# yangdongchao/RSTnet

Measured on NVIDIA H100. Metric: codec_frames_per_s, higher is better.
Workload: dtype f32

## Files before the change

### include/rstnet_b200.h

```cpp
#ifndef RSTNET_B200_H
#define RSTNET_B200_H

#include <stdint.h>

#ifdef __cplusplus
extern "C" {
#endif

typedef void* rstnet_stream_t;

enum { RSTNET_ACT_NONE = 0, RSTNET_ACT_ELU = 1, RSTNET_ACT_GELU = 2 };

int rstnet_version(void);
const char* rstnet_last_error(void);
int64_t rstnet_launch_count(void);
uint32_t rstnet_device_error_flags(int clear);

typedef struct {
  const float* A;
  int64_t a_batch_stride, a_row_stride;
  const float* Wt;
  const float* bias;
  const float* scale;
  const float* R;
  int64_t r_batch_stride, r_row_stride;
  float* C;
  int64_t c_batch_stride, c_row_stride;
  int32_t batch, rows, N, K;
  int32_t pre_act, post_act;
  int32_t taps;
  int64_t tap_stride;
} rstnet_gemm_rows_args;
int rstnet_gemm_rows_f32(const rstnet_gemm_rows_args* args, rstnet_stream_t stream);

typedef struct rstnet_tc_plan rstnet_tc_plan;
typedef struct {
  const float* A;
  int64_t a_i_stride, a_o_stride;
  int32_t a_c_extent, a_i_extent, a_o_extent;
  int32_t taps, tap_di, tap_do, o_mul;
  const float* W;
  const float* W_lo;
  int32_t N, Kc;
  int32_t I_out, O_out;
  float* C;
  int64_t c_i_stride, c_o_stride, c_split_stride;
  const float* R;
  int64_t r_i_stride, r_o_stride, r_split_stride;
  const float* bias;
  const float* scale;
  int32_t n_split;
  int32_t pre_act, post_act, precision;
  float* C2;
  int32_t act2;
} rstnet_tc_gemm_desc;
int rstnet_tc_gemm_create(const rstnet_tc_gemm_desc* desc, rstnet_tc_plan** out);
int rstnet_tc_gemm_run(const rstnet_tc_plan* plan, rstnet_stream_t stream);
void rstnet_tc_gemm_destroy(rstnet_tc_plan* plan);
int rstnet_tc_gemm_grid(const rstnet_tc_plan* plan, int32_t* grid_x, int32_t* grid_y, int32_t* tile_n);
int rstnet_tc_gemm_create_ex(const rstnet_tc_gemm_desc* desc, int32_t kpair, rstnet_tc_plan** out);
int rstnet_tc_gemm_kpair(const rstnet_tc_plan* plan, int32_t* on);
typedef struct rstnet_tc_resblock_plan rstnet_tc_resblock_plan;
typedef struct {
  const float* Y;
  int64_t y_i_stride, y_o_stride;
  int32_t channels;
  int32_t I_out, O_out, y_rows;
  const float* W1;
  const float* W1_lo;
  const float* b1;
  const float* W2;
  const float* W2_lo;
  const float* b2;
  float* out;
  int64_t out_i_stride, out_o_stride;
} rstnet_tc_resblock_desc;
int rstnet_tc_resblock_create(const rstnet_tc_resblock_desc* desc, rstnet_tc_resblock_plan** out);
int rstnet_tc_resblock_run(const rstnet_tc_resblock_plan* plan, rstnet_stream_t stream);
void rstnet_tc_resblock_destroy(rstnet_tc_resblock_plan* plan);

int rstnet_tf32_split_f32(const float* x, float* hi, float* lo, int64_t n, rstnet_stream_t stream);

int rstnet_conv1d_cin1_f32(const float* x, int64_t x_batch_stride, int64_t x_time_stride, const float* w, const float* bias,
                           float* out, float* out2 , int64_t out_batch_stride,
                           int64_t out_time_stride, int32_t batch, int32_t T, int32_t Cout, int32_t k,
                           int32_t post_act, int32_t act2, rstnet_stream_t stream);

int rstnet_conv1d_cout1_f32(const float* x, int64_t x_batch_stride, int64_t x_time_stride, const float* w,
                            const float* bias, float* out, int64_t out_batch_stride, int32_t batch,
                            int32_t T, int32_t Cin, int32_t k, rstnet_stream_t stream);

int rstnet_convtr1d_depthwise_f32(const float* x, int64_t x_batch_stride, int64_t x_time_stride,
                                  const float* w, float* out, int64_t out_batch_stride,
                                  int64_t out_time_stride, int32_t batch, int32_t T, int32_t C,
                                  int32_t stride, rstnet_stream_t stream);

int rstnet_rows_fill_f32(float* buf, int64_t batch_stride, int32_t batch, int32_t C, int32_t row0,
                         int32_t nrows, int32_t mode, int32_t src_row, const int64_t* only_if_zero,
                         int32_t only_if_zero_stride ,
                         int32_t channels_per_stream, rstnet_stream_t stream);
int rstnet_rows_fill_tail_f32(float* buf, int64_t batch_stride, int32_t batch, int32_t C, int32_t row0, int32_t nrows,
                              int32_t mode, const int64_t* valid, int64_t valid_div, int32_t channels_per_stream,
                              rstnet_stream_t stream);
typedef struct {
  float* buf;
  int64_t batch_stride;
  int32_t C, src_row, dst_row, nrows;
  int32_t cps;
  int32_t reserved;
} rstnet_row_copy;
int rstnet_rows_copy_table_f32(const rstnet_row_copy* table_dev, int32_t n_entries, int32_t batch,
                               const int64_t* active, rstnet_stream_t stream);
int rstnet_counter_add(int64_t* counter, int64_t delta, int32_t n, const int64_t* active ,
                       rstnet_stream_t stream);
int rstnet_counter_add_rows(int64_t* counter, const int64_t* delta, int32_t n, rstnet_stream_t stream);

int rstnet_layer_norm_f32(const float* x, int64_t x_batch_stride, const float* weight, const float* bias,
                          float* y, int32_t batch, int32_t rows_per_batch, int32_t dim, float eps,
                          rstnet_stream_t stream);

int rstnet_rope_kv_append_f32(float* qkv, int64_t q_batch_stride, int64_t q_time_stride, float* kv,
                              const int64_t* offset, int32_t offset_stride, const float* freqs, int32_t batch,
                              int32_t T, int32_t H, int32_t D, int32_t cap, rstnet_stream_t stream);
int rstnet_ring_attention_f32(const float* qkv, int64_t q_batch_stride, int64_t q_time_stride,
                              const float* kv, const int64_t* offset, int32_t offset_stride, float* out,
                              int64_t o_batch_stride, int64_t o_time_stride, int32_t batch, int32_t T,
                              int32_t H, int32_t D, int32_t cap, int32_t context, int32_t linear,
                              rstnet_stream_t stream);
int rstnet_rope_ring_attention_f32(const float* qkv, int64_t q_batch_stride, int64_t q_time_stride, float* kv,
                                   const int64_t* offset, int32_t offset_stride, const float* freqs, float* out,
                                   int64_t o_batch_stride, int64_t o_time_stride, int32_t batch, int32_t T, int32_t H,
                                   int32_t D, int32_t cap, int32_t context, rstnet_stream_t stream);

int64_t rstnet_rvq_encode_workspace(int64_t N, int32_t n_q, int32_t dim, int32_t bins);
int rstnet_rvq_encode_f32(const float* x, int64_t ldx, const float* E, const float* Et,
                          const float* enorm, int64_t* codes, void* work, int64_t N, int32_t T,
                          int32_t n_q, int32_t n_q_semantic, int32_t dim, int32_t bins,
                          int32_t time_major, rstnet_stream_t stream);
int rstnet_rvq_decode_gather_f32(const int64_t* codes, const float* E, float* q, int64_t N, int32_t T,
                                 int32_t n_q, int32_t n_q_semantic, int32_t dim, int32_t bins,
                                 int32_t time_major, rstnet_stream_t stream);

#define RSTNET_RESAMPLE_MAX_TABLE_BYTES (48 * 1024)
int rstnet_resample_f32(const float* x, int64_t x_row_stride, int64_t x_len, int64_t x_shift, const float* taps,
                        const int32_t* start, int32_t n, int32_t o, int32_t S, int32_t start_max, float* out,
                        int64_t out_row_stride, int64_t out_len, int32_t rows, rstnet_stream_t stream);

#define RSTNET_STFT_FRAMES_PER_BLOCK 16
int64_t rstnet_stft_loss_workspace(int32_t clips, int64_t max_len, int32_t hop);
int rstnet_stft_loss_sums_f32(const float* ref, const float* deg, const int64_t* offsets, const int64_t* lengths,
                              int32_t clips, int64_t min_len, int64_t max_len, int32_t n_fft, int32_t hop, int32_t win,
                              const float* twiddle, const float* window, double* sums, int32_t n_res, int32_t res,
                              void* ws, int64_t ws_bytes, rstnet_stream_t stream);

#define RSTNET_SISNR_SAMPLES_PER_BLOCK 8192
int64_t rstnet_sisnr_moments_workspace(int32_t clips, int64_t max_len);
int rstnet_sisnr_moments_f32(const float* ref, const float* deg, const int64_t* offsets, const int64_t* lengths,
                             int32_t clips, int64_t max_len, double* moments, void* ws, int64_t ws_bytes,
                             rstnet_stream_t stream);


typedef struct rstnet_skinny_plan rstnet_skinny_plan;
int64_t rstnet_skinny_gemm_workspace(int32_t M, int32_t N, int32_t max_splits);
int rstnet_skinny_gemm_create(const void* X, const void* W, const void* R, void* out, float* partial_ws,
                              int32_t M, int32_t N, int32_t K, int32_t max_splits, rstnet_skinny_plan** plan);
int rstnet_skinny_gemm_create_fused(const void* X, const void* W, const void* R, void* out, float* partial_ws,
                                    int32_t M, int32_t N, int32_t K, int32_t max_splits, int32_t fin_mode,
                                    const void* norm_w, void* aux_out, float eps, int32_t kyutai,
                                    rstnet_skinny_plan** plan);
int rstnet_skinny_gemm_run(const rstnet_skinny_plan* plan, rstnet_stream_t stream);
void rstnet_skinny_gemm_destroy(rstnet_skinny_plan* plan);

int rstnet_lm_embed_sum_bf16(const int64_t* seq, int32_t seq_stride, const void* wte, int64_t wte_rows,
                             const void* const* tables_dev, int64_t table_rows, int32_t n_q, int32_t E, void* x, int32_t rows,
                             rstnet_stream_t stream);
int rstnet_lm_embed_rows_bf16(const int64_t* ids, int32_t id_stride, const void* table, int64_t table_rows, int32_t D,
                              void* out, int32_t rows, rstnet_stream_t stream);
int rstnet_lm_rms_norm_bf16(const void* x, const void* w, void* y, int32_t rows, int32_t dim, float eps, int32_t kyutai,
                            rstnet_stream_t stream);
int rstnet_lm_rope_kv_append_bf16(const void* qkv, const void* cos_tab, const void* sin_tab, int64_t rope_rows, int32_t rope_n,
                                  const int64_t* offset, int32_t offset_stride ,
                                  const int32_t* row_stream, const int32_t* row_tl, void* q_out, void* kv, int32_t rows,
                                  int32_t B, int32_t n_head, int32_t n_kv, int32_t hs, int32_t cap, rstnet_stream_t stream);
#define RSTNET_KV_LOG2_PAGE_MIN 4
#define RSTNET_KV_LOG2_PAGE_MAX 12
int rstnet_lm_rope_kv_append_paged_bf16(const void* qkv, const void* cos_tab, const void* sin_tab, int64_t rope_rows,
                                        int32_t rope_n, const int64_t* offset, int32_t offset_stride, const int32_t* row_stream,
                                        const int32_t* row_tl, void* q_out, void* kv, int32_t rows, int32_t B, int32_t n_head,
                                        int32_t n_kv, int32_t hs, int32_t cap, const int32_t* page_table, int32_t pages_stride,
                                        int32_t log2_page, rstnet_stream_t stream);
int rstnet_lm_rope_pair_kv_append_bf16(const void* qkv, const int64_t* offset, int32_t offset_stride, void* q_out, void* kv,
                                       int32_t rows, int32_t B, int32_t H, int32_t hd, int32_t cap, const float* freqs,
                                       rstnet_stream_t stream);
int rstnet_lm_ring_decode_attention_bf16(const void* q, const void* kv, const int64_t* offset, int32_t offset_stride,
                                         const int32_t* row_stream, const int32_t* row_tl, void* out, int32_t rows, int32_t B,
                                         int32_t n_head, int32_t n_kv, int32_t hs, int32_t cap, int32_t context,
                                         rstnet_stream_t stream);
int rstnet_lm_paged_decode_attention_bf16(const void* q, const void* kv, const int64_t* offset, int32_t offset_stride,
                                          const int32_t* row_stream, const int32_t* row_tl, void* out, int32_t rows, int32_t B,
                                          int32_t n_head, int32_t n_kv, int32_t hs, int32_t cap, int32_t context,
                                          const int32_t* page_table, int32_t pages_stride, int32_t log2_page,
                                          rstnet_stream_t stream);
int rstnet_lm_silu_mul_bf16(const void* ab, void* out, int32_t M, int32_t I, rstnet_stream_t stream);
int rstnet_lm_depth_attention_bf16(const void* qkv, void* kvd, void* out, int32_t B, int32_t H, int32_t hd, int32_t cap,
                                   int32_t step, int32_t ring_quirk, rstnet_stream_t stream);
int rstnet_lm_sample_params_bf16(const void* logits, int32_t rows, int32_t V, int32_t n_valid, const int32_t* n_valid_rows,
                                 int32_t n_valid_stride, int32_t top_k, float temp, float top_p, const int32_t* top_k_rows,
                                 const float* temp_rows, const float* top_p_rows, int32_t param_stride, uint32_t seed,
                                 const int64_t* step_counter, const int64_t* step_rows, const uint32_t* key_rows,
                                 int64_t* tokens, int32_t tok_stride, rstnet_stream_t stream);

int rstnet_lm_cross_entropy_bf16(const void* logits, int64_t row_stride, int32_t rows, int32_t V, int32_t groups,
                                 const int64_t* labels, const int64_t* ignore_ids, const float* weights,
                                 const int32_t* row_slot, int32_t n_slots, float* nll, int32_t* pred, double* acc,
                                 rstnet_stream_t stream);

int rstnet_lm_delay_cache_in(int64_t* cache, const int64_t* off, const int64_t* active, const int64_t* delays,
                             const int64_t* user, int32_t user_stride, int64_t* seq, int32_t seq_stride, int32_t B, int32_t K,
                             int32_t dep_q, int32_t CT, int64_t text_init, int64_t audio_init, rstnet_stream_t stream);
int rstnet_lm_delay_cache_out(int64_t* cache, int64_t* off, const int64_t* active, const int64_t* delays,
                              const int64_t* tokens, int32_t tok_stride, int64_t* out, int32_t out_stride, int64_t* valid,
                              int32_t B, int32_t K, int32_t dep_q, int32_t CT, int32_t max_delay, rstnet_stream_t stream);

#ifdef __cplusplus
}
#endif
#endif
```

### rstnet_b200/_lib.py

```python
from __future__ import annotations

import ctypes as C
import os

_HERE = os.path.dirname(os.path.abspath(__file__))
LIB_PATH = os.path.join(_HERE, "lib", "librstnet_b200.so")

ACT_NONE, ACT_ELU, ACT_GELU = 0, 1, 2

SYMBOLS = [
    "rstnet_version", "rstnet_last_error", "rstnet_launch_count", "rstnet_device_error_flags",
    "rstnet_gemm_rows_f32", "rstnet_tc_gemm_create", "rstnet_tc_gemm_run", "rstnet_tc_gemm_destroy", "rstnet_tc_gemm_grid",
    "rstnet_tc_gemm_create_ex", "rstnet_tc_gemm_kpair",
    "rstnet_tc_resblock_create", "rstnet_tc_resblock_run", "rstnet_tc_resblock_destroy", "rstnet_tf32_split_f32", "rstnet_conv1d_cin1_f32", "rstnet_conv1d_cout1_f32",
    "rstnet_convtr1d_depthwise_f32", "rstnet_rows_fill_f32", "rstnet_rows_copy_table_f32",
    "rstnet_counter_add", "rstnet_layer_norm_f32", "rstnet_rope_kv_append_f32",
    "rstnet_ring_attention_f32", "rstnet_rope_ring_attention_f32", "rstnet_rvq_encode_workspace", "rstnet_rvq_encode_f32",
    "rstnet_rvq_decode_gather_f32",
    "rstnet_skinny_gemm_workspace", "rstnet_skinny_gemm_create", "rstnet_skinny_gemm_create_fused", "rstnet_skinny_gemm_run", "rstnet_skinny_gemm_destroy",
    "rstnet_lm_embed_sum_bf16", "rstnet_lm_embed_rows_bf16", "rstnet_lm_rms_norm_bf16", "rstnet_lm_rope_kv_append_bf16",
    "rstnet_lm_rope_pair_kv_append_bf16",
    "rstnet_lm_ring_decode_attention_bf16", "rstnet_lm_silu_mul_bf16", "rstnet_lm_depth_attention_bf16",
    "rstnet_resample_f32", "rstnet_lm_delay_cache_in", "rstnet_lm_delay_cache_out", "rstnet_counter_add_rows",
    "rstnet_lm_cross_entropy_bf16", "rstnet_rows_fill_tail_f32", "rstnet_lm_sample_params_bf16",
    "rstnet_lm_rope_kv_append_paged_bf16", "rstnet_lm_paged_decode_attention_bf16",
    "rstnet_stft_loss_workspace", "rstnet_stft_loss_sums_f32", "rstnet_sisnr_moments_workspace", "rstnet_sisnr_moments_f32",
]

KV_LOG2_PAGE_MIN, KV_LOG2_PAGE_MAX = 4, 12

RESAMPLE_MAX_TABLE_BYTES = 48 * 1024

STFT_FRAMES_PER_BLOCK = 16
SISNR_SAMPLES_PER_BLOCK = 8192


class GemmRowsArgs(C.Structure):
    _fields_ = [
        ("A", C.c_void_p), ("a_batch_stride", C.c_int64), ("a_row_stride", C.c_int64),
        ("Wt", C.c_void_p), ("bias", C.c_void_p), ("scale", C.c_void_p),
        ("R", C.c_void_p), ("r_batch_stride", C.c_int64), ("r_row_stride", C.c_int64),
        ("C", C.c_void_p), ("c_batch_stride", C.c_int64), ("c_row_stride", C.c_int64),
        ("batch", C.c_int32), ("rows", C.c_int32), ("N", C.c_int32), ("K", C.c_int32),
        ("pre_act", C.c_int32), ("post_act", C.c_int32), ("taps", C.c_int32), ("tap_stride", C.c_int64),
    ]


class TcGemmDesc(C.Structure):
    _fields_ = [
        ("A", C.c_void_p), ("a_i_stride", C.c_int64), ("a_o_stride", C.c_int64),
        ("a_c_extent", C.c_int32), ("a_i_extent", C.c_int32), ("a_o_extent", C.c_int32),
        ("taps", C.c_int32), ("tap_di", C.c_int32), ("tap_do", C.c_int32), ("o_mul", C.c_int32),
        ("W", C.c_void_p), ("W_lo", C.c_void_p), ("N", C.c_int32), ("Kc", C.c_int32), ("I_out", C.c_int32), ("O_out", C.c_int32),
        ("C", C.c_void_p), ("c_i_stride", C.c_int64), ("c_o_stride", C.c_int64), ("c_split_stride", C.c_int64),
        ("R", C.c_void_p), ("r_i_stride", C.c_int64), ("r_o_stride", C.c_int64), ("r_split_stride", C.c_int64),
        ("bias", C.c_void_p), ("scale", C.c_void_p),
        ("n_split", C.c_int32), ("pre_act", C.c_int32), ("post_act", C.c_int32), ("precision", C.c_int32),
        ("C2", C.c_void_p), ("act2", C.c_int32),
    ]


class TcResblockDesc(C.Structure):
    _fields_ = [
        ("Y", C.c_void_p), ("y_i_stride", C.c_int64), ("y_o_stride", C.c_int64),
        ("channels", C.c_int32), ("I_out", C.c_int32), ("O_out", C.c_int32), ("y_rows", C.c_int32),
        ("W1", C.c_void_p), ("W1_lo", C.c_void_p), ("b1", C.c_void_p),
        ("W2", C.c_void_p), ("W2_lo", C.c_void_p), ("b2", C.c_void_p),
        ("out", C.c_void_p), ("out_i_stride", C.c_int64), ("out_o_stride", C.c_int64),
    ]


class RowCopy(C.Structure):
    _fields_ = [("buf", C.c_void_p), ("batch_stride", C.c_int64), ("C", C.c_int32), ("src_row", C.c_int32),
                ("dst_row", C.c_int32), ("nrows", C.c_int32), ("cps", C.c_int32), ("reserved", C.c_int32)]


class RstnetError(RuntimeError):
    pass


_lib = None


def lib() -> C.CDLL:
    global _lib
    if _lib is not None:
        return _lib
    if not os.path.exists(LIB_PATH):
        raise RstnetError(
            f"{LIB_PATH} not found: the CUDA extension is not built. Run `python -m rstnet_b200.build` "
            "(there is no CPU fallback).")
    from . import build as _build
    stamp = os.path.join(os.path.dirname(LIB_PATH), "build.sha256")
    if os.path.isdir(_build.CSRC) and (not os.path.exists(stamp) or open(stamp).read().strip() != _build._digest()):
        raise RstnetError(
            f"{LIB_PATH} is stale (built from different sources than rstnet_b200/csrc + include/). "
            "Run `python -m rstnet_b200.build`.")
    L = C.CDLL(LIB_PATH)
    vp, i32, i64, f32 = C.c_void_p, C.c_int32, C.c_int64, C.c_float
    L.rstnet_version.restype = C.c_int
    L.rstnet_last_error.restype = C.c_char_p
    L.rstnet_launch_count.restype = i64
    L.rstnet_gemm_rows_f32.argtypes = [C.POINTER(GemmRowsArgs), vp]
    L.rstnet_tc_gemm_create.argtypes = [C.POINTER(TcGemmDesc), C.POINTER(C.c_void_p)]
    L.rstnet_tc_gemm_run.argtypes = [vp, vp]
    L.rstnet_tc_gemm_destroy.argtypes = [vp]
    L.rstnet_tc_gemm_destroy.restype = None
    L.rstnet_tc_gemm_grid.argtypes = [vp, C.POINTER(i32), C.POINTER(i32), C.POINTER(i32)]
    L.rstnet_tc_gemm_create_ex.argtypes = [C.POINTER(TcGemmDesc), i32, C.POINTER(C.c_void_p)]
    L.rstnet_tc_gemm_kpair.argtypes = [vp, C.POINTER(i32)]
    L.rstnet_tc_resblock_create.argtypes = [C.POINTER(TcResblockDesc), C.POINTER(C.c_void_p)]
    L.rstnet_tc_resblock_run.argtypes = [vp, vp]
    L.rstnet_tc_resblock_destroy.argtypes = [vp]
    L.rstnet_tc_resblock_destroy.restype = None
    L.rstnet_tf32_split_f32.argtypes = [vp, vp, vp, i64, vp]
    L.rstnet_conv1d_cin1_f32.argtypes = [vp, i64, i64, vp, vp, vp, vp, i64, i64, i32, i32, i32, i32, i32, i32, vp]
    L.rstnet_conv1d_cout1_f32.argtypes = [vp, i64, i64, vp, vp, vp, i64, i32, i32, i32, i32, vp]
    L.rstnet_convtr1d_depthwise_f32.argtypes = [vp, i64, i64, vp, vp, i64, i64, i32, i32, i32, i32, vp]
    L.rstnet_rows_fill_f32.argtypes = [vp, i64, i32, i32, i32, i32, i32, i32, vp, i32, i32, vp]
    L.rstnet_rows_fill_tail_f32.argtypes = [vp, i64, i32, i32, i32, i32, i32, vp, i64, i32, vp]
    L.rstnet_rows_copy_table_f32.argtypes = [vp, i32, i32, vp, vp]
    L.rstnet_counter_add.argtypes = [vp, i64, i32, vp, vp]
    L.rstnet_layer_norm_f32.argtypes = [vp, i64, vp, vp, vp, i32, i32, i32, f32, vp]
    L.rstnet_rope_kv_append_f32.argtypes = [vp, i64, i64, vp, vp, i32, vp, i32, i32, i32, i32, i32, vp]
    L.rstnet_ring_attention_f32.argtypes = [vp, i64, i64, vp, vp, i32, vp, i64, i64, i32, i32, i32, i32, i32, i32, i32, vp]
    L.rstnet_rope_ring_attention_f32.argtypes = [vp, i64, i64, vp, vp, i32, vp, vp, i64, i64, i32, i32, i32, i32, i32, i32, vp]
    L.rstnet_rvq_encode_workspace.argtypes = [i64, i32, i32, i32]
    L.rstnet_rvq_encode_workspace.restype = i64
    L.rstnet_rvq_encode_f32.argtypes = [vp, i64, vp, vp, vp, vp, vp, i64, i32, i32, i32, i32, i32, i32, vp]
    L.rstnet_rvq_decode_gather_f32.argtypes = [vp, vp, vp, i64, i32, i32, i32, i32, i32, i32, vp]
    L.rstnet_skinny_gemm_workspace.argtypes = [i32, i32, i32]
    L.rstnet_skinny_gemm_workspace.restype = i64
    L.rstnet_skinny_gemm_create.argtypes = [vp, vp, vp, vp, vp, i32, i32, i32, i32, C.POINTER(C.c_void_p)]
    L.rstnet_skinny_gemm_create_fused.argtypes = [vp, vp, vp, vp, vp, i32, i32, i32, i32, i32, vp, vp, f32, i32, C.POINTER(C.c_void_p)]
    L.rstnet_skinny_gemm_run.argtypes = [vp, vp]
    L.rstnet_skinny_gemm_destroy.argtypes = [vp]
    L.rstnet_skinny_gemm_destroy.restype = None
    L.rstnet_lm_embed_sum_bf16.argtypes = [vp, i32, vp, i64, vp, i64, i32, i32, vp, i32, vp]
    L.rstnet_lm_embed_rows_bf16.argtypes = [vp, i32, vp, i64, i32, vp, i32, vp]
    L.rstnet_device_error_flags.argtypes = [i32]
    L.rstnet_device_error_flags.restype = C.c_uint32
    L.rstnet_lm_rms_norm_bf16.argtypes = [vp, vp, vp, i32, i32, f32, i32, vp]
    L.rstnet_lm_rope_kv_append_bf16.argtypes = [vp, vp, vp, i64, i32, vp, i32, vp, vp, vp, vp, i32, i32, i32, i32, i32, i32, vp]
    L.rstnet_lm_rope_pair_kv_append_bf16.argtypes = [vp, vp, i32, vp, vp, i32, i32, i32, i32, i32, vp, vp]
    L.rstnet_lm_ring_decode_attention_bf16.argtypes = [vp, vp, vp, i32, vp, vp, vp, i32, i32, i32, i32, i32, i32, i32, vp]
    L.rstnet_lm_rope_kv_append_paged_bf16.argtypes = [vp, vp, vp, i64, i32, vp, i32, vp, vp, vp, vp, i32, i32, i32, i32, i32, i32,
                                                      vp, i32, i32, vp]
    L.rstnet_lm_paged_decode_attention_bf16.argtypes = [vp, vp, vp, i32, vp, vp, vp, i32, i32, i32, i32, i32, i32, i32, vp, i32, i32,
                                                        vp]
    L.rstnet_lm_silu_mul_bf16.argtypes = [vp, vp, i32, i32, vp]
    L.rstnet_lm_depth_attention_bf16.argtypes = [vp, vp, vp, i32, i32, i32, i32, i32, i32, vp]
    L.rstnet_resample_f32.argtypes = [vp, i64, i64, i64, vp, vp, i32, i32, i32, i32, vp, i64, i64, i32, vp]
    L.rstnet_lm_delay_cache_in.argtypes = [vp, vp, vp, vp, vp, i32, vp, i32, i32, i32, i32, i32, i64, i64, vp]
    L.rstnet_lm_delay_cache_out.argtypes = [vp, vp, vp, vp, vp, i32, vp, i32, vp, i32, i32, i32, i32, i32, vp]
    L.rstnet_counter_add_rows.argtypes = [vp, vp, i32, vp]
    L.rstnet_lm_cross_entropy_bf16.argtypes = [vp, i64, i32, i32, i32, vp, vp, vp, vp, i32, vp, vp, vp, vp]
    L.rstnet_lm_sample_params_bf16.argtypes = [vp, i32, i32, i32, vp, i32, i32, f32, f32, vp, vp, vp, i32, C.c_uint32, vp, vp, vp,
                                               vp, i32, vp]
    L.rstnet_stft_loss_workspace.argtypes = [i32, i64, i32]
    L.rstnet_stft_loss_workspace.restype = i64
    L.rstnet_stft_loss_sums_f32.argtypes = [vp, vp, vp, vp, i32, i64, i64, i32, i32, i32, vp, vp, vp, i32, i32, vp, i64, vp]
    L.rstnet_sisnr_moments_workspace.argtypes = [i32, i64]
    L.rstnet_sisnr_moments_workspace.restype = i64
    L.rstnet_sisnr_moments_f32.argtypes = [vp, vp, vp, vp, i32, i64, vp, vp, i64, vp]
    for name in SYMBOLS:
        fn = getattr(L, name)
        if fn.restype is C.c_int and name not in ("rstnet_version",):
            pass
    _lib = L
    return L


def check(rc: int, what: str = "") -> None:
    if rc != 0:
        msg = lib().rstnet_last_error()
        raise RstnetError(f"{what or 'rstnet call'} failed (rc={rc}): {msg.decode() if msg else '?'}")


def launch_count() -> int:
    return int(lib().rstnet_launch_count())
```

### rstnet_b200/csrc/gemm_tc.cu

```cuda
#include <cstdlib>

#include "common.cuh"
#include "tc_common.cuh"
#include "../../include/rstnet_b200.h"

namespace rstnet {
extern void count_launch();
using namespace tc;

constexpr int TC_BM = 128;
constexpr int TC_BKE = 32;
constexpr int TC_A_BYTES = TC_BM * 128;
constexpr int TC_CONSUMER_WARPS = 8;
constexpr int TC_THREADS = 32 * TC_CONSUMER_WARPS + 32;
constexpr int TC_CHUNK_STAGES = 4;

struct TcParams {
  float* C;
  float* C2;
  int act2;
  long long c_i_stride, c_o_stride, c_split_stride;
  const float* R;
  long long r_i_stride, r_o_stride, r_split_stride;
  const float* bias;
  const float* scale;
  int n_split;
  int I_out, O_out, N, Kc;
  int taps, tap_di, tap_do, o_mul, kchunks;
  int pre_act, post_act, i_tiles;
  int m_tiles, n_tiles;
  int kpair;
};

template <int BN, int PREC>
struct TcCfg {
  static constexpr bool SPLIT = PREC == 0;
  static constexpr int B_BYTES = BN * 128;
  static constexpr int STAGE_BYTES = TC_A_BYTES + B_BYTES * (SPLIT ? 2 : 1);
  static constexpr int STAGES = (200 * 1024 / STAGE_BYTES) > 8 ? 8 : (200 * 1024 / STAGE_BYTES);
  static constexpr int SMEM_BYTES = STAGES * STAGE_BYTES + 1024  + 256 ;
  static constexpr int Q_PIECES = BN / 32;
  static_assert(STAGES % 2 == 0 && 2 * Q_PIECES <= STAGES, "K-pair rings and queue");
};

__device__ __forceinline__ float tf32_rna(float x) {
  const uint32_t u = __float_as_uint(x);
  return __uint_as_float((x != x ? u | 0x00400000u : u + 0x1000u) & 0xFFFFE000u);
}
__device__ __forceinline__ float tf32_rna_lo(float x, float hi) {
  const float d = x - hi;
  return d != d ? 0.f : __uint_as_float((__float_as_uint(d) + 0x1000u) & 0xFFFFE000u);
}

__device__ __forceinline__ float act_tc(float x, int act) {
  if (act == ACT_ELU) return elu_fast(x);
  if (act == ACT_GELU) return gelu_f(x);
  return x;
}

template <bool SPLIT, bool PRE_ELU>
__device__ __forceinline__ void tc_build_a(uint32_t st, uint32_t a_row, uint32_t a_sw, uint32_t (&ah)[4][4], uint32_t (&al)[4][4]) {
#pragma unroll
  for (int k = 0; k < 4; ++k) {
#pragma unroll
    for (int e = 0; e < 4; ++e) {
      const uint32_t chunk = (uint32_t)(2 * k + (e >> 1));
      float v;
      asm volatile("ld.shared.f32 %0, [%1];" : "=f"(v) : "r"(st + a_row + (e & 1) * 1024u + ((chunk ^ a_sw) << 4)));
      if (PRE_ELU) {
        const float e = __expf(v) - 1.f;
        v = v > 0.f ? v : e;
      }
      if (SPLIT) {
        const bool nonfinite = !(fabsf(v) < INFINITY);
        const float h = nonfinite ? 0.f : __uint_as_float((__float_as_uint(v) + 0x1000u) & 0xFFFFE000u);
        const float d = v - h;
        ah[k][e] = __float_as_uint(h);
        al[k][e] = (__float_as_uint(d) + (nonfinite ? 0u : 0x1000u)) & 0xFFFFE000u;
      } else {
        ah[k][e] = __float_as_uint(tf32_rna(v));
      }
    }
  }
}

template <int BN, bool SPLIT>
__device__ __forceinline__ void tc_mma_stage(float (&d0)[BN / 2], float (&d1)[BN / 2], const uint32_t (&ah)[4][4],
                                             const uint32_t (&al)[4][4], uint64_t db, uint64_t dbl, bool first) {
#pragma unroll
  for (int k = 0; k < 4; ++k) {
    const uint32_t acc_in = (first && k == 0) ? 0u : 1u;
    wgmma_tf32_rs<BN>(d0, ah[k], db + (uint64_t)(2 * k), acc_in);
    if (SPLIT) {
      wgmma_tf32_rs<BN>(d1, al[k], db + (uint64_t)(2 * k), acc_in);
      wgmma_tf32_rs<BN>(d1, ah[k], dbl + (uint64_t)(2 * k), 1u);
    }
  }
}

template <int BN, int PREC, bool PRE_ELU, bool KP>
__global__ void __launch_bounds__(TC_THREADS, 1)
gemm_tc_kernel(const __grid_constant__ CUtensorMap tmA, const __grid_constant__ CUtensorMap tmW,
               const __grid_constant__ CUtensorMap tmWlo, const TcParams p) {
  using Cfg = TcCfg<BN, PREC>;
  constexpr int S = Cfg::STAGES;
  constexpr int CH = TC_CHUNK_STAGES;
  constexpr int NR = BN / 2;
  extern __shared__ uint8_t smem_raw[];
  uint8_t* smem = smem_raw + ((1024u - (smem_u32(smem_raw) & 1023u)) & 1023u);
  uint64_t* full = reinterpret_cast<uint64_t*>(smem + S * Cfg::STAGE_BYTES);
  uint64_t* empty = full + S;
  uint64_t* qfull = empty + S;
  uint64_t* qempty = qfull + 2;
  const int warp = threadIdx.x / 32, lane = threadIdx.x % 32;
  const int total_k = p.taps * p.kchunks;
  const int total_tiles = p.m_tiles * p.n_tiles;
  const int bm = KP ? TC_BM / 2 : TC_BM;
  const int R = KP ? S / 2 : S;

  if (threadIdx.x == 0) {
    for (int s = 0; s < S; ++s) {
      mbar_init(&full[s], 1);
      mbar_init(&empty[s], KP ? TC_CONSUMER_WARPS / 2 : TC_CONSUMER_WARPS);
    }
    for (int q = 0; q < 2; ++q) {
      mbar_init(&qfull[q], 128);
      mbar_init(&qempty[q], 128);
    }
    fence_barrier_init();
  }
  __syncthreads();

  if (warp == TC_CONSUMER_WARPS) {
    if (elect_one()) {
      tma_prefetch_desc(&tmA);
      tma_prefetch_desc(&tmW);
      if (Cfg::SPLIT) tma_prefetch_desc(&tmWlo);
      int pos0 = 0, ph0 = 0, pos1 = 0, ph1 = 0;
      for (int t = blockIdx.x; t < total_tiles; t += gridDim.x) {
        const int nt = t % p.n_tiles, mt = t / p.n_tiles;
        const int i0 = (mt % p.i_tiles) * bm, ot = mt / p.i_tiles, n0 = nt * BN;
        for (int kit = 0; kit < total_k; ++kit) {
          const int w = KP ? (kit / TC_CHUNK_STAGES) & 1 : 0;
          const int pos = w ? pos1 : pos0, ph = w ? ph1 : ph0;
          const int s = w * R + pos;
          const int npos = pos + 1 == R ? 0 : pos + 1, nph = ph ^ (npos == 0);
          if (w) { pos1 = npos; ph1 = nph; } else { pos0 = npos; ph0 = nph; }
          mbar_wait(&empty[s], ph ^ 1);
          const int tap = kit / p.kchunks, kc = kit % p.kchunks;
          uint8_t* st = smem + s * Cfg::STAGE_BYTES;
          mbar_arrive_expect_tx(&full[s], Cfg::STAGE_BYTES - (TC_BM - bm) * 128);
          tma_load_3d(st, &tmA, &full[s], kc * TC_BKE, i0 + tap * p.tap_di, ot * p.o_mul + tap * p.tap_do);
          tma_load_2d(st + TC_A_BYTES, &tmW, &full[s], kit * TC_BKE, n0);
          if (Cfg::SPLIT) tma_load_2d(st + TC_A_BYTES + Cfg::B_BYTES, &tmWlo, &full[s], kit * TC_BKE, n0);
        }
      }
    }
    return;
  }

  const int wg = warp / 4, wq = warp % 4, gq = lane / 4, tq = lane % 4;
  const int r0 = (KP ? 0 : wg * 64) + wq * 16 + gq;
  const uint32_t a_row = (uint32_t)r0 * 128u + (uint32_t)tq * 4u, a_sw = (uint32_t)(r0 & 7);
  const uint32_t smem0 = smem_u32(smem);
  float acc[NR], d0[NR], d1[NR];
#pragma unroll
  for (int j = 0; j < NR; ++j) d0[j] = d1[j] = 0.f;
  const int nch = (total_k + CH - 1) / CH;
  const bool sender = KP && wg == 1;
  auto qel = [&](int q, int j) {
    return reinterpret_cast<float*>(smem + (q * Cfg::Q_PIECES + j / 16) * Cfg::STAGE_BYTES + TC_A_BYTES / 2) +
           (j % 16) * 128 + (threadIdx.x & 127);
  };
  int qn = 0;
  auto take_queued = [&]() {
    mbar_wait(&qfull[qn & 1], (qn >> 1) & 1);
#pragma unroll
    for (int j = 0; j < NR; ++j) acc[j] += *qel(qn & 1, j);
    mbar_arrive(&qempty[qn & 1]);
    ++qn;
  };
  const int base = KP ? wg * R : 0;
  int pos = 0, ph = 0;
  for (int t = blockIdx.x; t < total_tiles; t += gridDim.x) {
    const int nt = t % p.n_tiles, mt = t / p.n_tiles;
    const int i0 = (mt % p.i_tiles) * bm, ot = mt / p.i_tiles, n0 = nt * BN;
#pragma unroll
    for (int j = 0; j < NR; ++j) acc[j] = 0.f;
    for (int c = KP ? wg : 0; c < nch; c += KP ? 2 : 1) {
      const int k0 = c * CH;
      const int nst = total_k - k0 < CH ? total_k - k0 : CH;
      for (int u = 0; u < nst; ++u) {
        const int s = base + pos;
        mbar_wait(&full[s], ph);
        const uint32_t st = smem0 + (uint32_t)(s * Cfg::STAGE_BYTES);
        uint32_t ah[4][4], al[4][4];
        tc_build_a<Cfg::SPLIT, PRE_ELU>(st, a_row, a_sw, ah, al);
        const uint64_t db = gmma_desc_sw128(st + TC_A_BYTES);
        const uint64_t dbl = gmma_desc_sw128(st + TC_A_BYTES + Cfg::B_BYTES);
        wgmma_fence();
        tc_mma_stage<BN, Cfg::SPLIT>(d0, d1, ah, al, db, dbl, u == 0);
        wgmma_commit();
        wgmma_wait<0>();
        __syncwarp();
        if (lane == 0) mbar_arrive(&empty[s]);
        pos = pos + 1 == R ? 0 : pos + 1;
        ph ^= pos == 0;
      }
      fence_acc(d0);
      if (Cfg::SPLIT) fence_acc(d1);
      if (sender) {
        mbar_wait(&qempty[qn & 1], ((qn >> 1) & 1) ^ 1);
#pragma unroll
        for (int j = 0; j < NR; ++j) *qel(qn & 1, j) = Cfg::SPLIT ? d0[j] + d1[j] : d0[j];
        mbar_arrive(&qfull[qn & 1]);
        ++qn;
      } else {
        if (KP && c > 0) take_queued();
#pragma unroll
        for (int j = 0; j < NR; ++j) acc[j] += Cfg::SPLIT ? d0[j] + d1[j] : d0[j];
      }
    }
    if (KP && !sender && nch % 2 == 0) take_queued();
    if (sender) continue;
#pragma unroll
    for (int h = 0; h < 2; ++h) {
      const int i = i0 + r0 + 8 * h;
      if (i >= p.I_out) continue;
      float* crow = p.C + (long long)ot * p.c_o_stride + (long long)i * p.c_i_stride;
      float* crow2 = p.C2 ? p.C2 + (long long)ot * p.c_o_stride + (long long)i * p.c_i_stride : nullptr;
      const float* rrow = p.R ? p.R + (long long)ot * p.r_o_stride + (long long)i * p.r_i_stride : nullptr;
#pragma unroll
      for (int b = 0; b < BN / 8; ++b) {
        const int n = n0 + 8 * b + 2 * tq;
        if (n < p.N) {
          float2 v = make_float2(acc[4 * b + 2 * h], acc[4 * b + 2 * h + 1]);
          if (p.bias) {
            const float2 bb = *reinterpret_cast<const float2*>(p.bias + n);
            v.x += bb.x; v.y += bb.y;
          }
          if (p.scale) {
            const float2 ss = *reinterpret_cast<const float2*>(p.scale + n);
            v.x *= ss.x; v.y *= ss.y;
          }
          long long coff = n, roff = n;
          if (p.n_split > 0) {
            const int j = n / p.n_split, co = n % p.n_split;
            coff = (long long)j * p.c_split_stride + co;
            roff = (long long)j * p.r_split_stride + co;
          }
          if (rrow) {
            const float2 rr = *reinterpret_cast<const float2*>(rrow + roff);
            v.x += rr.x; v.y += rr.y;
          }
          if (crow2)
            *reinterpret_cast<float2*>(crow2 + coff) = make_float2(act_tc(v.x, p.act2), act_tc(v.y, p.act2));
          *reinterpret_cast<float2*>(crow + coff) = make_float2(act_tc(v.x, p.post_act), act_tc(v.y, p.post_act));
        }
      }
    }
  }
}

constexpr int RB_B_BYTES = 64 * 128;
constexpr int RB_STAGE_BYTES = TC_A_BYTES + 2 * RB_B_BYTES;
constexpr int RB_STAGES = 6;

struct RbParams {
  float* out;
  long long o_i_stride, o_o_stride;
  const float* b1;
  const float* b2;
  int I_out, i_tiles, m_tiles;
};

template <int C>
struct RbCfg {
  static constexpr int N1 = C / 2;
  static constexpr int KCH = C / 32;
  static constexpr int P1 = 3 * KCH;
  static constexpr int NS = C / 64;
  static constexpr int K2 = N1 / 32;
  static constexpr int H_BYTES = K2 * TC_A_BYTES;
  static constexpr int SMEM_BYTES = RB_STAGES * RB_STAGE_BYTES + H_BYTES + 1024  + 256 ;
  static constexpr bool ring_ok() {
    for (int j = 0; j < NS; ++j)
      for (int kc = 0; kc < KCH; ++kc)
        if ((P1 + j) % RB_STAGES == (2 * KCH + kc) % RB_STAGES) return false;
    return RB_STAGES >= KCH + NS;
  }
  static_assert(ring_ok(), "ring too small for the held residual stages");
  static_assert(K2 * 2 * RB_B_BYTES <= RB_STAGE_BYTES, "a phase-2 slice must fit one stage");
};

template <int C>
__global__ void __launch_bounds__(TC_THREADS, 1)
resblock_tc_kernel(const __grid_constant__ CUtensorMap tmY, const __grid_constant__ CUtensorMap tmW1,
                   const __grid_constant__ CUtensorMap tmW1lo, const __grid_constant__ CUtensorMap tmW2,
                   const __grid_constant__ CUtensorMap tmW2lo, const RbParams p) {
  using Cfg = RbCfg<C>;
  constexpr int S = RB_STAGES;
  constexpr int CH = TC_CHUNK_STAGES;
  constexpr int N1 = Cfg::N1, NR1 = N1 / 2, KCH = Cfg::KCH, P1 = Cfg::P1;
  extern __shared__ uint8_t smem_raw[];
  uint8_t* smem = smem_raw + ((1024u - (smem_u32(smem_raw) & 1023u)) & 1023u);
  uint8_t* hs = smem + S * RB_STAGE_BYTES;
  uint64_t* full = reinterpret_cast<uint64_t*>(hs + Cfg::H_BYTES);
  uint64_t* empty = full + S;
  const int warp = threadIdx.x / 32, lane = threadIdx.x % 32;

  if (threadIdx.x == 0) {
    for (int s = 0; s < S; ++s) {
      mbar_init(&full[s], 1);
      mbar_init(&empty[s], TC_CONSUMER_WARPS);
    }
    fence_barrier_init();
  }
  __syncthreads();

  if (warp == TC_CONSUMER_WARPS) {
    if (elect_one()) {
      tma_prefetch_desc(&tmY);
      tma_prefetch_desc(&tmW1);
      tma_prefetch_desc(&tmW1lo);
      tma_prefetch_desc(&tmW2);
      tma_prefetch_desc(&tmW2lo);
      int g = 0;
      for (int t = blockIdx.x; t < p.m_tiles; t += gridDim.x) {
        const int i0 = (t % p.i_tiles) * TC_BM, ot = t / p.i_tiles;
        for (int kit = 0; kit < P1; ++kit, ++g) {
          const int s = g % S;
          mbar_wait(&empty[s], ((g / S) & 1) ^ 1);
          const int tap = kit / KCH, kc = kit % KCH;
          uint8_t* st = smem + s * RB_STAGE_BYTES;
          mbar_arrive_expect_tx(&full[s], TC_A_BYTES + 2 * N1 * 128);
          tma_load_3d(st, &tmY, &full[s], kc * TC_BKE, i0, ot + tap);
          tma_load_2d(st + TC_A_BYTES, &tmW1, &full[s], kit * TC_BKE, 0);
          tma_load_2d(st + TC_A_BYTES + RB_B_BYTES, &tmW1lo, &full[s], kit * TC_BKE, 0);
        }
        for (int ns = 0; ns < Cfg::NS; ++ns, ++g) {
          const int s = g % S;
          mbar_wait(&empty[s], ((g / S) & 1) ^ 1);
          uint8_t* st = smem + s * RB_STAGE_BYTES;
          mbar_arrive_expect_tx(&full[s], Cfg::K2 * 2 * RB_B_BYTES);
#pragma unroll
          for (int kc = 0; kc < Cfg::K2; ++kc) {
            tma_load_2d(st + kc * 2 * RB_B_BYTES, &tmW2, &full[s], kc * TC_BKE, ns * 64);
            tma_load_2d(st + kc * 2 * RB_B_BYTES + RB_B_BYTES, &tmW2lo, &full[s], kc * TC_BKE, ns * 64);
          }
        }
      }
    }
    return;
  }

  const int wg = warp / 4, wq = warp % 4, gq = lane / 4, tq = lane % 4;
  const int r0 = wg * 64 + wq * 16 + gq;
  const uint32_t a_row = (uint32_t)r0 * 128u + (uint32_t)tq * 4u, a_sw = (uint32_t)(r0 & 7);
  const uint32_t smem0 = smem_u32(smem), hs0 = smem_u32(hs);
  int g = 0;
  for (int t = blockIdx.x; t < p.m_tiles; t += gridDim.x) {
    const int i0 = (t % p.i_tiles) * TC_BM, ot = t / p.i_tiles;
    const int g_res = g + 2 * KCH;
    {
      float acc[NR1], d0[NR1], d1[NR1];
#pragma unroll
      for (int j = 0; j < NR1; ++j) acc[j] = d0[j] = d1[j] = 0.f;
      for (int k0 = 0; k0 < P1; k0 += CH) {
        const int nst = P1 - k0 < CH ? P1 - k0 : CH;
        for (int u = 0; u < nst; ++u, ++g) {
          const int s = g % S;
          mbar_wait(&full[s], (g / S) & 1);
          const uint32_t st = smem0 + (uint32_t)(s * RB_STAGE_BYTES);
          uint32_t ah[4][4], al[4][4];
          tc_build_a<true, true>(st, a_row, a_sw, ah, al);
          wgmma_fence();
          tc_mma_stage<N1, true>(d0, d1, ah, al, gmma_desc_sw128(st + TC_A_BYTES), gmma_desc_sw128(st + TC_A_BYTES + RB_B_BYTES),
                                 u == 0);
          wgmma_commit();
          wgmma_wait<0>();
          __syncwarp();
          if (lane == 0 && k0 + u < 2 * KCH) mbar_arrive(&empty[s]);
        }
        fence_acc(d0);
        fence_acc(d1);
#pragma unroll
        for (int j = 0; j < NR1; ++j) acc[j] += d0[j] + d1[j];
      }
      named_bar_sync(1 + wg, 128);
#pragma unroll
      for (int hh = 0; hh < 2; ++hh) {
        const int r = r0 + 8 * hh;
#pragma unroll
        for (int b = 0; b < N1 / 8; ++b) {
          const int n = 8 * b + 2 * tq;
          const float2 bb = *reinterpret_cast<const float2*>(p.b1 + n);
          float2 v = make_float2(acc[4 * b + 2 * hh], acc[4 * b + 2 * hh + 1]);
          v.x += bb.x; v.y += bb.y;
          const uint32_t cc = (uint32_t)(n % 32);
          const uint32_t addr = hs0 + (uint32_t)(n / 32) * TC_A_BYTES + (uint32_t)r * 128u + (((cc >> 2) ^ (uint32_t)(r & 7)) << 4) +
                                (cc & 3u) * 4u;
          asm volatile("st.shared.v2.f32 [%0], {%1, %2};" ::"r"(addr), "f"(act_tc(v.x, ACT_ELU)), "f"(act_tc(v.y, ACT_ELU))
                       : "memory");
        }
      }
      named_bar_sync(1 + wg, 128);
    }
    for (int ns = 0; ns < Cfg::NS; ++ns, ++g) {
      const int s = g % S;
      mbar_wait(&full[s], (g / S) & 1);
      const uint32_t st = smem0 + (uint32_t)(s * RB_STAGE_BYTES);
      float acc[32], d0[32], d1[32];
#pragma unroll
      for (int j = 0; j < 32; ++j) d0[j] = d1[j] = 0.f;
#pragma unroll
      for (int kc = 0; kc < Cfg::K2; ++kc) {
        uint32_t ah[4][4], al[4][4];
        tc_build_a<true, false>(hs0 + (uint32_t)(kc * TC_A_BYTES), a_row, a_sw, ah, al);
        const uint32_t wst = st + (uint32_t)(kc * 2 * RB_B_BYTES);
        wgmma_fence();
        tc_mma_stage<64, true>(d0, d1, ah, al, gmma_desc_sw128(wst), gmma_desc_sw128(wst + RB_B_BYTES), kc == 0);
        wgmma_commit();
        wgmma_wait<0>();
      }
      __syncwarp();
      if (lane == 0) mbar_arrive(&empty[s]);
      fence_acc(d0);
      fence_acc(d1);
#pragma unroll
      for (int j = 0; j < 32; ++j) {
        acc[j] = 0.f;
        acc[j] += d0[j] + d1[j];
      }
#pragma unroll
      for (int hh = 0; hh < 2; ++hh) {
        const int r = r0 + 8 * hh;
        const int i = i0 + r;
        if (i >= p.I_out) continue;
        float* orow = p.out + (long long)ot * p.o_o_stride + (long long)i * p.o_i_stride;
#pragma unroll
        for (int b = 0; b < 8; ++b) {
          const int n = ns * 64 + 8 * b + 2 * tq;
          const float2 bb = *reinterpret_cast<const float2*>(p.b2 + n);
          float2 v = make_float2(acc[4 * b + 2 * hh], acc[4 * b + 2 * hh + 1]);
          v.x += bb.x; v.y += bb.y;
          const uint32_t cc = (uint32_t)(n % 32);
          const int rs = (g_res + n / 32) % S;
          const float2 rr = *reinterpret_cast<const float2*>(smem + rs * RB_STAGE_BYTES + r * 128 +
                                                             (((cc >> 2) ^ (uint32_t)(r & 7)) << 4) + (cc & 3u) * 4u);
          v.x += rr.x; v.y += rr.y;
          *reinterpret_cast<float2*>(orow + n) = make_float2(act_tc(v.x, ACT_ELU), act_tc(v.y, ACT_ELU));
        }
      }
      __syncwarp();
      if (lane == 0) {
        mbar_arrive(&empty[(g_res + 2 * ns) % S]);
        mbar_arrive(&empty[(g_res + 2 * ns + 1) % S]);
      }
    }
  }
}

typedef CUresult (*EncodeTiledFn)(CUtensorMap*, CUtensorMapDataType, cuuint32_t, void*, const cuuint64_t*, const cuuint64_t*,
                                  const cuuint32_t*, const cuuint32_t*, CUtensorMapInterleave, CUtensorMapSwizzle,
                                  CUtensorMapL2promotion, CUtensorMapFloatOOBfill);

static EncodeTiledFn get_encode_fn() {
  static EncodeTiledFn fn = nullptr;
  if (!fn) {
    void* p = nullptr;
    cudaDriverEntryPointQueryResult q;
    if (cudaGetDriverEntryPoint("cuTensorMapEncodeTiled", &p, cudaEnableDefault, &q) == cudaSuccess && p) fn = (EncodeTiledFn)p;
  }
  return fn;
}

}
using namespace rstnet;

struct rstnet_tc_plan {
  CUtensorMap tmA, tmW, tmWlo;
  TcParams p;
  dim3 grid;
  int bn, prec;
};

template <int BN, int PREC, bool PRE_ELU, bool KP>
static int tc_launch(const rstnet_tc_plan* pl, cudaStream_t st) {
  using Cfg = TcCfg<BN, PREC>;
  static unsigned long long attr = 0;
  smem_optin(gemm_tc_kernel<BN, PREC, PRE_ELU, KP>, Cfg::SMEM_BYTES, attr);
  gemm_tc_kernel<BN, PREC, PRE_ELU, KP><<<pl->grid, TC_THREADS, Cfg::SMEM_BYTES, st>>>(pl->tmA, pl->tmW, pl->tmWlo, pl->p);
  count_launch();
  return check_launch("gemm_tc");
}

template <int BN, int PREC>
static int tc_launch_mode(const rstnet_tc_plan* pl, cudaStream_t st) {
  const bool elu = pl->p.pre_act == ACT_ELU;
  if (pl->p.kpair) return elu ? tc_launch<BN, PREC, true, true>(pl, st) : tc_launch<BN, PREC, false, true>(pl, st);
  return elu ? tc_launch<BN, PREC, true, false>(pl, st) : tc_launch<BN, PREC, false, false>(pl, st);
}

extern "C" int rstnet_tc_gemm_create_ex(const rstnet_tc_gemm_desc* d, int32_t kpair, rstnet_tc_plan** out) {
  RSTNET_REQUIRE(d && out, "tc_gemm_create: null argument");
  RSTNET_REQUIRE(kpair >= -1 && kpair <= 1, "tc_gemm_create: kpair must be -1 (auto), 0 or 1 (got %d)", kpair);
  RSTNET_REQUIRE(d->A && d->W && d->C, "tc_gemm_create: null tensor pointer");
  RSTNET_REQUIRE(d->precision != 0 || d->W_lo, "tc_gemm_create: precision 0 (3xTF32) needs W_lo");
  RSTNET_REQUIRE(d->Kc > 0 && d->Kc % TC_BKE == 0, "tc_gemm_create: Kc (%d) must be a multiple of %d", d->Kc, TC_BKE);
  RSTNET_REQUIRE(d->N > 0 && d->N % 4 == 0, "tc_gemm_create: N (%d) must be a multiple of 4", d->N);
  RSTNET_REQUIRE(d->taps >= 1 && d->I_out > 0 && d->O_out > 0, "tc_gemm_create: bad shape");
  RSTNET_REQUIRE(d->precision == 0 || d->precision == 1, "tc_gemm_create: precision must be 0 (3xTF32) or 1 (TF32)");
  RSTNET_REQUIRE(d->pre_act == ACT_NONE || d->pre_act == ACT_ELU, "tc_gemm_create: pre_act must be NONE or ELU (got %d)", d->pre_act);
  RSTNET_REQUIRE((uintptr_t)d->A % 16 == 0 && (uintptr_t)d->W % 16 == 0 && (uintptr_t)d->C % 16 == 0 &&
                     d->a_i_stride % 4 == 0 && d->a_o_stride % 4 == 0 && d->c_i_stride % 4 == 0 && d->c_o_stride % 4 == 0 &&
                     d->c_split_stride % 4 == 0 && d->n_split % 4 == 0,
                 "tc_gemm_create: 16-byte alignment required");
  EncodeTiledFn enc = get_encode_fn();
  RSTNET_REQUIRE(enc != nullptr, "tc_gemm_create: cuTensorMapEncodeTiled unavailable (no CUDA driver?)");
  rstnet_tc_plan* pl = new rstnet_tc_plan();
  const int N = d->N;
  const int sms = sm_count();
  pl->bn = N >= 64 ? 64 : 32;
  const int i_tiles = ceil_div(d->I_out, TC_BM);
  {
    const long long mt = (long long)i_tiles * d->O_out;
    const long long t64 = mt * ceil_div(N, 64), t32 = mt * ceil_div(N, 32);
    if (pl->bn == 64 && ((t32 + sms - 1) / sms) * 2 <= ((t64 + sms - 1) / sms) * 3) pl->bn = 32;
  }
  pl->prec = d->precision;
  const int n_tiles = ceil_div(N, pl->bn);
  if (kpair < 0) {
    const long long total_k = (long long)d->taps * (d->Kc / TC_BKE);
    const long long t128 = (long long)i_tiles * d->O_out * n_tiles, t64 = (long long)ceil_div(d->I_out, TC_BM / 2) * d->O_out * n_tiles;
    const long long pair_k = (total_k + 2 * TC_CHUNK_STAGES - 1) / (2 * TC_CHUNK_STAGES) * TC_CHUNK_STAGES;
    kpair = t128 <= sms && ((t64 + sms - 1) / sms) * pair_k < total_k;
  }
  const int bm = kpair ? TC_BM / 2 : TC_BM;
  {
    cuuint64_t gdim[3] = {(cuuint64_t)d->a_c_extent, (cuuint64_t)d->a_i_extent, (cuuint64_t)d->a_o_extent};
    cuuint64_t gstr[2] = {(cuuint64_t)d->a_i_stride * 4, (cuuint64_t)d->a_o_stride * 4};
    cuuint32_t box[3] = {TC_BKE, (cuuint32_t)bm, 1};
    cuuint32_t estr[3] = {1, 1, 1};
    CUresult r = enc(&pl->tmA, CU_TENSOR_MAP_DATA_TYPE_FLOAT32, 3, (void*)d->A, gdim, gstr, box, estr, CU_TENSOR_MAP_INTERLEAVE_NONE,
                     CU_TENSOR_MAP_SWIZZLE_128B, CU_TENSOR_MAP_L2_PROMOTION_L2_128B, CU_TENSOR_MAP_FLOAT_OOB_FILL_NONE);
    if (r != CUDA_SUCCESS) {
      delete pl;
      set_error("tc_gemm_create: cuTensorMapEncodeTiled(A) failed with %d", (int)r);
      return 3;
    }
  }
  {
    cuuint64_t gdim[2] = {(cuuint64_t)d->taps * d->Kc, (cuuint64_t)N};
    cuuint64_t gstr[1] = {(cuuint64_t)d->taps * d->Kc * 4};
    cuuint32_t box[2] = {TC_BKE, (cuuint32_t)pl->bn};
    cuuint32_t estr[2] = {1, 1};
    CUresult r = enc(&pl->tmW, CU_TENSOR_MAP_DATA_TYPE_FLOAT32, 2, (void*)d->W, gdim, gstr, box, estr, CU_TENSOR_MAP_INTERLEAVE_NONE,
                     CU_TENSOR_MAP_SWIZZLE_128B, CU_TENSOR_MAP_L2_PROMOTION_L2_256B, CU_TENSOR_MAP_FLOAT_OOB_FILL_NONE);
    if (r == CUDA_SUCCESS && d->W_lo)
      r = enc(&pl->tmWlo, CU_TENSOR_MAP_DATA_TYPE_FLOAT32, 2, (void*)d->W_lo, gdim, gstr, box, estr, CU_TENSOR_MAP_INTERLEAVE_NONE,
              CU_TENSOR_MAP_SWIZZLE_128B, CU_TENSOR_MAP_L2_PROMOTION_L2_256B, CU_TENSOR_MAP_FLOAT_OOB_FILL_NONE);
    else
      pl->tmWlo = pl->tmW;
    if (r != CUDA_SUCCESS) {
      delete pl;
      set_error("tc_gemm_create: cuTensorMapEncodeTiled(W) failed with %d", (int)r);
      return 3;
    }
  }
  TcParams& p = pl->p;
  p.C2 = d->C2; p.act2 = d->act2;
  p.C = d->C; p.c_i_stride = d->c_i_stride; p.c_o_stride = d->c_o_stride; p.c_split_stride = d->c_split_stride;
  p.R = d->R; p.r_i_stride = d->r_i_stride; p.r_o_stride = d->r_o_stride; p.r_split_stride = d->r_split_stride;
  p.bias = d->bias; p.scale = d->scale; p.n_split = d->n_split;
  p.I_out = d->I_out; p.O_out = d->O_out; p.N = N; p.Kc = d->Kc;
  p.taps = d->taps; p.tap_di = d->tap_di; p.tap_do = d->tap_do; p.o_mul = d->o_mul; p.kchunks = d->Kc / TC_BKE;
  p.pre_act = d->pre_act; p.post_act = d->post_act;
  p.kpair = kpair;
  p.i_tiles = ceil_div(d->I_out, bm);
  p.m_tiles = p.i_tiles * d->O_out;
  p.n_tiles = n_tiles;
  const long long tiles = (long long)p.m_tiles * p.n_tiles;
  pl->grid = dim3((unsigned)(tiles < sms ? tiles : sms));
  *out = pl;
  return 0;
}

extern "C" int rstnet_tc_gemm_create(const rstnet_tc_gemm_desc* d, rstnet_tc_plan** out) {
  return rstnet_tc_gemm_create_ex(d, -1, out);
}

extern "C" int rstnet_tc_gemm_run(const rstnet_tc_plan* pl, rstnet_stream_t stream) {
  RSTNET_REQUIRE(pl != nullptr, "tc_gemm_run: null plan");
  cudaStream_t st = (cudaStream_t)stream;
  if (pl->prec == 0) return pl->bn == 64 ? tc_launch_mode<64, 0>(pl, st) : tc_launch_mode<32, 0>(pl, st);
  return pl->bn == 64 ? tc_launch_mode<64, 1>(pl, st) : tc_launch_mode<32, 1>(pl, st);
}

extern "C" void rstnet_tc_gemm_destroy(rstnet_tc_plan* pl) { delete pl; }

struct rstnet_tc_resblock_plan {
  CUtensorMap tmY, tmW1, tmW1lo, tmW2, tmW2lo;
  RbParams p;
  dim3 grid;
  int channels;
};

static int encode_2d(CUtensorMap* m, const float* base, int cols, int rows, int box_rows) {
  cuuint64_t gdim[2] = {(cuuint64_t)cols, (cuuint64_t)rows};
  cuuint64_t gstr[1] = {(cuuint64_t)cols * 4};
  cuuint32_t box[2] = {TC_BKE, (cuuint32_t)box_rows};
  cuuint32_t estr[2] = {1, 1};
  return (int)get_encode_fn()(m, CU_TENSOR_MAP_DATA_TYPE_FLOAT32, 2, (void*)base, gdim, gstr, box, estr, CU_TENSOR_MAP_INTERLEAVE_NONE,
                              CU_TENSOR_MAP_SWIZZLE_128B, CU_TENSOR_MAP_L2_PROMOTION_L2_256B, CU_TENSOR_MAP_FLOAT_OOB_FILL_NONE);
}

extern "C" int rstnet_tc_resblock_create(const rstnet_tc_resblock_desc* d, rstnet_tc_resblock_plan** out) {
  RSTNET_REQUIRE(d && out, "tc_resblock_create: null argument");
  RSTNET_REQUIRE(d->Y && d->W1 && d->W1_lo && d->b1 && d->W2 && d->W2_lo && d->b2 && d->out, "tc_resblock_create: null pointer");
  const int Cc = d->channels;
  RSTNET_REQUIRE(Cc == 64 || Cc == 128, "tc_resblock_create: channels must be 64 or 128 (got %d)", Cc);
  RSTNET_REQUIRE(d->I_out > 0 && d->O_out > 0 && d->y_rows >= d->O_out + 2, "tc_resblock_create: bad shape");
  RSTNET_REQUIRE((uintptr_t)d->Y % 16 == 0 && (uintptr_t)d->W1 % 16 == 0 && (uintptr_t)d->W1_lo % 16 == 0 && (uintptr_t)d->W2 % 16 == 0 &&
                     (uintptr_t)d->W2_lo % 16 == 0 && (uintptr_t)d->out % 16 == 0 && (uintptr_t)d->b1 % 8 == 0 &&
                     (uintptr_t)d->b2 % 8 == 0 && d->y_i_stride % 4 == 0 && d->y_o_stride % 4 == 0 && d->out_i_stride % 4 == 0 &&
                     d->out_o_stride % 4 == 0,
                 "tc_resblock_create: 16-byte alignment required");
  RSTNET_REQUIRE(get_encode_fn() != nullptr, "tc_resblock_create: cuTensorMapEncodeTiled unavailable (no CUDA driver?)");
  rstnet_tc_resblock_plan* pl = new rstnet_tc_resblock_plan();
  pl->channels = Cc;
  int r;
  {
    cuuint64_t gdim[3] = {(cuuint64_t)Cc, (cuuint64_t)d->I_out, (cuuint64_t)d->y_rows};
    cuuint64_t gstr[2] = {(cuuint64_t)d->y_i_stride * 4, (cuuint64_t)d->y_o_stride * 4};
    cuuint32_t box[3] = {TC_BKE, TC_BM, 1};
    cuuint32_t estr[3] = {1, 1, 1};
    r = (int)get_encode_fn()(&pl->tmY, CU_TENSOR_MAP_DATA_TYPE_FLOAT32, 3, (void*)d->Y, gdim, gstr, box, estr, CU_TENSOR_MAP_INTERLEAVE_NONE,
                             CU_TENSOR_MAP_SWIZZLE_128B, CU_TENSOR_MAP_L2_PROMOTION_L2_128B, CU_TENSOR_MAP_FLOAT_OOB_FILL_NONE);
  }
  if (r == CUDA_SUCCESS) r = encode_2d(&pl->tmW1, d->W1, 3 * Cc, Cc / 2, Cc / 2);
  if (r == CUDA_SUCCESS) r = encode_2d(&pl->tmW1lo, d->W1_lo, 3 * Cc, Cc / 2, Cc / 2);
  if (r == CUDA_SUCCESS) r = encode_2d(&pl->tmW2, d->W2, Cc / 2, Cc, 64);
  if (r == CUDA_SUCCESS) r = encode_2d(&pl->tmW2lo, d->W2_lo, Cc / 2, Cc, 64);
  if (r != CUDA_SUCCESS) {
    delete pl;
    set_error("tc_resblock_create: cuTensorMapEncodeTiled failed with %d", r);
    return 3;
  }
  RbParams& p = pl->p;
  p.out = d->out; p.o_i_stride = d->out_i_stride; p.o_o_stride = d->out_o_stride;
  p.b1 = d->b1; p.b2 = d->b2;
  p.I_out = d->I_out;
  p.i_tiles = ceil_div(d->I_out, TC_BM);
  p.m_tiles = p.i_tiles * d->O_out;
  const int sms = sm_count();
  pl->grid = dim3((unsigned)(p.m_tiles < sms ? p.m_tiles : sms));
  *out = pl;
  return 0;
}

template <int Cc>
static int rb_launch(const rstnet_tc_resblock_plan* pl, cudaStream_t st) {
  constexpr int smem = RbCfg<Cc>::SMEM_BYTES;
  static unsigned long long attr = 0;
  smem_optin(resblock_tc_kernel<Cc>, smem, attr);
  resblock_tc_kernel<Cc><<<pl->grid, TC_THREADS, smem, st>>>(pl->tmY, pl->tmW1, pl->tmW1lo, pl->tmW2, pl->tmW2lo, pl->p);
  count_launch();
  return check_launch("tc_resblock");
}

extern "C" int rstnet_tc_resblock_run(const rstnet_tc_resblock_plan* pl, rstnet_stream_t stream) {
  RSTNET_REQUIRE(pl != nullptr, "tc_resblock_run: null plan");
  cudaStream_t st = (cudaStream_t)stream;
  return pl->channels == 64 ? rb_launch<64>(pl, st) : rb_launch<128>(pl, st);
}

extern "C" void rstnet_tc_resblock_destroy(rstnet_tc_resblock_plan* pl) { delete pl; }
extern "C" int rstnet_tc_gemm_grid(const rstnet_tc_plan* pl, int32_t* gx, int32_t* gy, int32_t* bn) {
  if (!pl) return 1;
  *gx = ceil_div(pl->p.I_out, TC_BM) * pl->p.O_out; *gy = pl->p.n_tiles; *bn = pl->bn;
  return 0;
}
extern "C" int rstnet_tc_gemm_kpair(const rstnet_tc_plan* pl, int32_t* on) {
  if (!pl) return 1;
  *on = pl->p.kpair;
  return 0;
}

namespace rstnet {
__global__ void tf32_split_kernel(const float* __restrict__ x, float* __restrict__ hi, float* __restrict__ lo, long long n) {
  for (long long i = (long long)blockIdx.x * blockDim.x + threadIdx.x; i < n; i += (long long)gridDim.x * blockDim.x) {
    const float v = x[i], h = tf32_rna(v);
    hi[i] = h;
    lo[i] = tf32_rna_lo(v, h);
  }
}
}

extern "C" int rstnet_tf32_split_f32(const float* x, float* hi, float* lo, int64_t n, rstnet_stream_t stream) {
  RSTNET_REQUIRE(x && hi && lo, "tf32_split: null pointer");
  if (n <= 0) return 0;
  int g = ceil_div(n, 256);
  if (g > sm_count() * 8) g = sm_count() * 8;
  rstnet::tf32_split_kernel<<<g, 256, 0, (cudaStream_t)stream>>>(x, hi, lo, n);
  count_launch();
  return check_launch("tf32_split");
}
```

### rstnet_b200/ops.py

```python
from __future__ import annotations

import ctypes as C
from typing import Optional

import torch

from . import _lib
from ._lib import ACT_ELU, ACT_GELU, ACT_NONE, GemmRowsArgs, RowCopy, TcGemmDesc


def _stream() -> int:
    return torch.cuda.current_stream().cuda_stream


def _p(t: Optional[torch.Tensor]) -> Optional[int]:
    return None if t is None else t.data_ptr()


def _cuda(*ts):
    for t in ts:
        if t is not None and not t.is_cuda:
            raise _lib.RstnetError("rstnet_b200 ops need CUDA tensors (there is no CPU path)")


def gemm_rows(A: torch.Tensor, a_off: int, a_bs: int, a_rs: int, Wt: torch.Tensor, C_: torch.Tensor, c_off: int,
              c_bs: int, c_rs: int, batch: int, rows: int, *, bias=None, scale=None, R=None, r_off: int = 0,
              r_bs: int = 0, r_rs: int = 0, pre_act: int = ACT_NONE, post_act: int = ACT_NONE, taps: int = 1,
              tap_stride: int = 0) -> None:
    _cuda(A, Wt, C_, bias, scale, R)
    K, N = Wt.shape
    a = GemmRowsArgs()
    a.A = A.data_ptr() + 4 * a_off
    a.a_batch_stride, a.a_row_stride = a_bs, a_rs
    a.Wt = Wt.data_ptr()
    a.bias, a.scale = _p(bias), _p(scale)
    a.R = None if R is None else R.data_ptr() + 4 * r_off
    a.r_batch_stride, a.r_row_stride = r_bs, r_rs
    a.C = C_.data_ptr() + 4 * c_off
    a.c_batch_stride, a.c_row_stride = c_bs, c_rs
    a.batch, a.rows, a.N, a.K = batch, rows, N, K
    a.pre_act, a.post_act = pre_act, post_act
    a.taps, a.tap_stride = taps, tap_stride
    _lib.check(_lib.lib().rstnet_gemm_rows_f32(C.byref(a), _stream()), "gemm_rows_f32")


def tf32_split(w: torch.Tensor):
    _cuda(w)
    w = w.contiguous()
    both = torch.empty((2,) + tuple(w.shape), dtype=w.dtype, device=w.device)
    hi, lo = both[0], both[1]
    _lib.check(_lib.lib().rstnet_tf32_split_f32(w.data_ptr(), hi.data_ptr(), lo.data_ptr(), w.numel(), _stream()), "tf32_split")
    return hi, lo


class TcGemm:

    def __init__(self, A, a_off, a_i_stride, a_o_stride, a_c_extent, a_i_extent, a_o_extent, W, Kc, C_, c_off, c_i_stride,
                 c_o_stride, I_out, O_out, *, taps=1, tap_di=0, tap_do=0, o_mul=1, bias=None, scale=None, R=None, r_off=0,
                 r_i_stride=0, r_o_stride=0, n_split=0, c_split_stride=0, r_split_stride=0, pre_act=ACT_NONE,
                 post_act=ACT_NONE, precision=0, W_lo=None, C2=None, c2_off=0, act2=ACT_NONE):
        _cuda(A, W, C_, bias, scale, R, W_lo)
        N, Ktot = W.shape
        if precision == 0 and W_lo is None:
            W, W_lo = tf32_split(W)
        assert Ktot == taps * Kc, (Ktot, taps, Kc)
        d = TcGemmDesc()
        d.A = A.data_ptr() + 4 * a_off
        d.a_i_stride, d.a_o_stride = a_i_stride, a_o_stride
        d.a_c_extent, d.a_i_extent, d.a_o_extent = a_c_extent, a_i_extent, a_o_extent
        d.taps, d.tap_di, d.tap_do, d.o_mul = taps, tap_di, tap_do, o_mul
        d.W, d.W_lo, d.N, d.Kc, d.I_out, d.O_out = W.data_ptr(), _p(W_lo), N, Kc, I_out, O_out
        d.C = C_.data_ptr() + 4 * c_off
        d.c_i_stride, d.c_o_stride, d.c_split_stride = c_i_stride, c_o_stride, c_split_stride
        d.R = None if R is None else R.data_ptr() + 4 * r_off
        d.r_i_stride, d.r_o_stride, d.r_split_stride = r_i_stride, r_o_stride, r_split_stride
        d.bias, d.scale = _p(bias), _p(scale)
        d.n_split, d.pre_act, d.post_act, d.precision = n_split, pre_act, post_act, precision
        d.C2 = None if C2 is None else C2.data_ptr() + 4 * c2_off
        d.act2 = act2
        self._keep = (A, W, W_lo, C_, bias, scale, R, C2)
        self.flops = 2.0 * I_out * O_out * N * Ktot
        in_rows = min(a_o_extent, O_out * o_mul + (taps - 1) * max(tap_do, 0))
        n_out = I_out * O_out * N
        self.bytes = 4.0 * (a_c_extent * a_i_extent * in_rows + (2 if W_lo is not None else 1) * N * Ktot
                            + n_out * (2 if C2 is not None else 1) + (n_out if R is not None else 0))
        self._h = C.c_void_p()
        _lib.check(_lib.lib().rstnet_tc_gemm_create(C.byref(d), C.byref(self._h)), "tc_gemm_create")

    def run(self):
        _lib.check(_lib.lib().rstnet_tc_gemm_run(self._h, _stream()), "tc_gemm_run")

    def __del__(self):
        h = getattr(self, "_h", None)
        if h:
            try:
                _lib.lib().rstnet_tc_gemm_destroy(h)
            except Exception:
                pass
            self._h = None


class TcResblock:

    def __init__(self, Y, y_off, y_i_stride, y_o_stride, y_rows, I_out, O_out, W1, W1_lo, b1, W2, W2_lo, b2, out, out_off,
                 out_i_stride, out_o_stride):
        _cuda(Y, W1, W1_lo, b1, W2, W2_lo, b2, out)
        Cc = W2.shape[0]
        assert tuple(W1.shape) == (Cc // 2, 3 * Cc) and tuple(W2.shape) == (Cc, Cc // 2), (W1.shape, W2.shape)
        d = _lib.TcResblockDesc()
        d.Y = Y.data_ptr() + 4 * y_off
        d.y_i_stride, d.y_o_stride = y_i_stride, y_o_stride
        d.channels, d.I_out, d.O_out, d.y_rows = Cc, I_out, O_out, y_rows
        d.W1, d.W1_lo, d.b1 = W1.data_ptr(), W1_lo.data_ptr(), b1.data_ptr()
        d.W2, d.W2_lo, d.b2 = W2.data_ptr(), W2_lo.data_ptr(), b2.data_ptr()
        d.out = out.data_ptr() + 4 * out_off
        d.out_i_stride, d.out_o_stride = out_i_stride, out_o_stride
        self._keep = (Y, W1, W1_lo, b1, W2, W2_lo, b2, out)
        self.shape = dict(C=Cc, I=I_out, O=O_out)
        n = I_out * O_out
        self.flops = 2.0 * n * (W1.numel() + W2.numel())
        self.bytes = 4.0 * (Cc * I_out * (O_out + 2) + 2 * (W1.numel() + W2.numel()) + b1.numel() + b2.numel() + n * Cc)
        self._h = C.c_void_p()
        _lib.check(_lib.lib().rstnet_tc_resblock_create(C.byref(d), C.byref(self._h)), "tc_resblock_create")

    def run(self):
        _lib.check(_lib.lib().rstnet_tc_resblock_run(self._h, _stream()), "tc_resblock_run")

    def __del__(self):
        h = getattr(self, "_h", None)
        if h:
            try:
                _lib.lib().rstnet_tc_resblock_destroy(h)
            except Exception:
                pass
            self._h = None


def conv1d_cin1(x, x_bs, x_ts, w, bias, out, out_off, out_bs, out_ts, batch, T, Cout, k, post_act=ACT_NONE, out2=None,
                out2_off=0, act2=ACT_NONE):
    _cuda(x, w, out, out2)
    _lib.check(_lib.lib().rstnet_conv1d_cin1_f32(x.data_ptr(), x_bs, x_ts, w.data_ptr(), _p(bias), out.data_ptr() + 4 * out_off,
                                                 None if out2 is None else out2.data_ptr() + 4 * out2_off, out_bs, out_ts,
                                                 batch, T, Cout, k, post_act, act2, _stream()), "conv1d_cin1")


def conv1d_cout1(x, x_bs, x_ts, w, bias, out, out_bs, batch, T, Cin, k):
    _cuda(x, w, out)
    _lib.check(_lib.lib().rstnet_conv1d_cout1_f32(x.data_ptr(), x_bs, x_ts, w.data_ptr(), _p(bias), out.data_ptr(), out_bs,
                                                  batch, T, Cin, k, _stream()), "conv1d_cout1")


def convtr1d_depthwise(x, x_bs, x_ts, w, out, out_off, out_bs, out_ts, batch, T, Cch, stride):
    _cuda(x, w, out)
    _lib.check(_lib.lib().rstnet_convtr1d_depthwise_f32(x.data_ptr(), x_bs, x_ts, w.data_ptr(), out.data_ptr() + 4 * out_off,
                                                        out_bs, out_ts, batch, T, Cch, stride, _stream()), "convtr1d_depthwise")


def rows_fill(buf, bs, batch, Cch, row0, nrows, mode=0, src_row=0, only_if_zero=None, channels_per_stream=0):
    _cuda(buf)
    oz_stride = 1 if (only_if_zero is not None and only_if_zero.numel() > 1) else 0
    _lib.check(_lib.lib().rstnet_rows_fill_f32(buf.data_ptr(), bs, batch, Cch, row0, nrows, mode, src_row,
                                               _p(only_if_zero), oz_stride, channels_per_stream, _stream()), "rows_fill")


def rows_fill_tail(buf, bs, batch, Cch, row0, nrows, mode, valid, valid_div=1, channels_per_stream=0):
    _cuda(buf, valid)
    _lib.check(_lib.lib().rstnet_rows_fill_tail_f32(buf.data_ptr(), bs, batch, Cch, row0, nrows, mode, valid.data_ptr(), valid_div,
                                                    channels_per_stream, _stream()), "rows_fill_tail")


def rows_copy_table(table_dev: torch.Tensor, n_entries: int, batch: int, active: Optional[torch.Tensor] = None):
    _lib.check(_lib.lib().rstnet_rows_copy_table_f32(table_dev.data_ptr(), n_entries, batch, _p(active), _stream()), "rows_copy_table")


def make_copy_table(entries, device) -> torch.Tensor:
    arr = (RowCopy * len(entries))()
    for i, (t, bs, c, s, d, n, cps) in enumerate(entries):
        if n > 0 and not (s >= d):
            raise _lib.RstnetError("carry copy must move rows towards the front (src_row >= dst_row)")
        arr[i].buf, arr[i].batch_stride, arr[i].C, arr[i].src_row, arr[i].dst_row, arr[i].nrows = t.data_ptr(), bs, c, s, d, n
        arr[i].cps = cps
    raw = bytes(arr)
    return torch.frombuffer(bytearray(raw), dtype=torch.uint8).to(device)


def counter_add(counter: torch.Tensor, delta: int, active: Optional[torch.Tensor] = None):
    if active is not None and active.numel() != counter.numel():
        active = None
    _lib.check(_lib.lib().rstnet_counter_add(counter.data_ptr(), delta, counter.numel(), _p(active), _stream()), "counter_add")


def _ostride(offset: torch.Tensor) -> int:
    return 1 if offset.numel() > 1 else 0


def layer_norm(x, x_off, x_bs, w, b, y, batch, rows, dim, eps):
    _cuda(x, w, b, y)
    _lib.check(_lib.lib().rstnet_layer_norm_f32(x.data_ptr() + 4 * x_off, x_bs, w.data_ptr(), b.data_ptr(), y.data_ptr(),
                                                batch, rows, dim, eps, _stream()), "layer_norm")


def rope_kv_append(qkv, q_bs, q_ts, kv, offset, freqs, batch, T, H, D, cap):
    _cuda(qkv, kv, offset, freqs)
    _lib.check(_lib.lib().rstnet_rope_kv_append_f32(qkv.data_ptr(), q_bs, q_ts, kv.data_ptr(), offset.data_ptr(), _ostride(offset),
                                                    freqs.data_ptr(), batch, T, H, D, cap, _stream()), "rope_kv_append")


def rope_ring_attention(qkv, q_bs, q_ts, kv, offset, freqs, out, o_bs, o_ts, batch, T, H, D, cap, context):
    _cuda(qkv, kv, offset, freqs, out)
    _lib.check(_lib.lib().rstnet_rope_ring_attention_f32(qkv.data_ptr(), q_bs, q_ts, kv.data_ptr(), offset.data_ptr(), _ostride(offset),
                                                         freqs.data_ptr(), out.data_ptr(), o_bs, o_ts, batch, T, H, D, cap, context,
                                                         _stream()), "rope_ring_attention")


def ring_attention(qkv, q_bs, q_ts, kv, offset, out, o_bs, o_ts, batch, T, H, D, cap, context, linear):
    _cuda(qkv, kv, offset, out)
    _lib.check(_lib.lib().rstnet_ring_attention_f32(qkv.data_ptr(), q_bs, q_ts, kv.data_ptr(), offset.data_ptr(), _ostride(offset),
                                                    out.data_ptr(), o_bs, o_ts, batch, T, H, D, cap, context, int(linear),
                                                    _stream()), "ring_attention")


def rvq_encode_workspace(N, n_q, dim, bins) -> int:
    return int(_lib.lib().rstnet_rvq_encode_workspace(N, n_q, dim, bins))


def rvq_encode(x, ldx, E, Et, enorm, codes, work, N, T, n_q, ns, dim, bins, time_major=False):
    _cuda(x, E, Et, enorm, codes, work)
    _lib.check(_lib.lib().rstnet_rvq_encode_f32(x.data_ptr(), ldx, E.data_ptr(), Et.data_ptr(), enorm.data_ptr(),
                                                codes.data_ptr(), work.data_ptr(), N, T, n_q, ns, dim, bins, int(time_major),
                                                _stream()), "rvq_encode")


def rvq_decode_gather(codes, E, q, N, T, n_q, ns, dim, bins, time_major=False):
    _cuda(codes, E, q)
    _lib.check(_lib.lib().rstnet_rvq_decode_gather_f32(codes.data_ptr(), E.data_ptr(), q.data_ptr(), N, T, n_q, ns, dim,
                                                       bins, int(time_major), _stream()), "rvq_decode_gather")


def stft_loss_workspace(clips, max_len, hop) -> int:
    return int(_lib.lib().rstnet_stft_loss_workspace(clips, max_len, hop))


def stft_loss_sums(ref, deg, offsets, lengths, clips, min_len, max_len, n_fft, hop, win, twiddle, window, sums, n_res, res,
                   ws):
    _cuda(ref, deg, offsets, lengths, twiddle, window, sums, ws)
    _lib.check(_lib.lib().rstnet_stft_loss_sums_f32(ref.data_ptr(), deg.data_ptr(), offsets.data_ptr(), lengths.data_ptr(),
                                                    clips, min_len, max_len, n_fft, hop, win, twiddle.data_ptr(),
                                                    window.data_ptr(), sums.data_ptr(), n_res, res, ws.data_ptr(),
                                                    ws.numel() * ws.element_size(), _stream()), "stft_loss_sums")


def sisnr_moments_workspace(clips, max_len) -> int:
    return int(_lib.lib().rstnet_sisnr_moments_workspace(clips, max_len))


def sisnr_moments(ref, deg, offsets, lengths, clips, max_len, moments, ws):
    _cuda(ref, deg, offsets, lengths, moments, ws)
    _lib.check(_lib.lib().rstnet_sisnr_moments_f32(ref.data_ptr(), deg.data_ptr(), offsets.data_ptr(), lengths.data_ptr(),
                                                   clips, max_len, moments.data_ptr(), ws.data_ptr(),
                                                   ws.numel() * ws.element_size(), _stream()), "sisnr_moments")
```

Before: 44500.

## Add two-CTA-per-SM variants of TC GEMM and resblock kernels for short-K shapes

Adds occupancy-2 variants of the warp-specialized TF32 GEMM (BN=32, 4 stages) and the 64-channel resblock kernel (3 stages, phase-2 split into 32-column halves). Both shrink shared memory so two CTAs fit per SM, and the grid is sized to twice the SM count. Plans pick these automatically when there are many tiles and the K loop is short, so prologue and epilogue latency of one CTA can overlap with another's work. The cost is a shallower TMA pipeline and extra register pressure from the launch bounds.

```diff
diff --git a/include/rstnet_b200.h b/include/rstnet_b200.h
--- a/include/rstnet_b200.h
+++ b/include/rstnet_b200.h
@@ -60,6 +60,8 @@
 int rstnet_tc_gemm_grid(const rstnet_tc_plan* plan, int32_t* grid_x, int32_t* grid_y, int32_t* tile_n);
 int rstnet_tc_gemm_create_ex(const rstnet_tc_gemm_desc* desc, int32_t kpair, rstnet_tc_plan** out);
 int rstnet_tc_gemm_kpair(const rstnet_tc_plan* plan, int32_t* on);
+int rstnet_tc_gemm_create_ex2(const rstnet_tc_gemm_desc* desc, int32_t kpair, int32_t occ2, rstnet_tc_plan** out);
+int rstnet_tc_gemm_occ2(const rstnet_tc_plan* plan, int32_t* on);
 typedef struct rstnet_tc_resblock_plan rstnet_tc_resblock_plan;
 typedef struct {
   const float* Y;
@@ -78,6 +80,8 @@
 int rstnet_tc_resblock_create(const rstnet_tc_resblock_desc* desc, rstnet_tc_resblock_plan** out);
 int rstnet_tc_resblock_run(const rstnet_tc_resblock_plan* plan, rstnet_stream_t stream);
 void rstnet_tc_resblock_destroy(rstnet_tc_resblock_plan* plan);
+int rstnet_tc_resblock_create_ex(const rstnet_tc_resblock_desc* desc, int32_t occ2, rstnet_tc_resblock_plan** out);
+int rstnet_tc_resblock_occ2(const rstnet_tc_resblock_plan* plan, int32_t* on);
 
 int rstnet_tf32_split_f32(const float* x, float* hi, float* lo, int64_t n, rstnet_stream_t stream);
 
diff --git a/rstnet_b200/_lib.py b/rstnet_b200/_lib.py
--- a/rstnet_b200/_lib.py
+++ b/rstnet_b200/_lib.py
@@ -11,8 +11,8 @@
 SYMBOLS = [
     "rstnet_version", "rstnet_last_error", "rstnet_launch_count", "rstnet_device_error_flags",
     "rstnet_gemm_rows_f32", "rstnet_tc_gemm_create", "rstnet_tc_gemm_run", "rstnet_tc_gemm_destroy", "rstnet_tc_gemm_grid",
-    "rstnet_tc_gemm_create_ex", "rstnet_tc_gemm_kpair",
-    "rstnet_tc_resblock_create", "rstnet_tc_resblock_run", "rstnet_tc_resblock_destroy", "rstnet_tf32_split_f32", "rstnet_conv1d_cin1_f32", "rstnet_conv1d_cout1_f32",
+    "rstnet_tc_gemm_create_ex", "rstnet_tc_gemm_kpair", "rstnet_tc_gemm_create_ex2", "rstnet_tc_gemm_occ2",
+    "rstnet_tc_resblock_create", "rstnet_tc_resblock_create_ex", "rstnet_tc_resblock_occ2", "rstnet_tc_resblock_run", "rstnet_tc_resblock_destroy", "rstnet_tf32_split_f32", "rstnet_conv1d_cin1_f32", "rstnet_conv1d_cout1_f32",
     "rstnet_convtr1d_depthwise_f32", "rstnet_rows_fill_f32", "rstnet_rows_copy_table_f32",
     "rstnet_counter_add", "rstnet_layer_norm_f32", "rstnet_rope_kv_append_f32",
     "rstnet_ring_attention_f32", "rstnet_rope_ring_attention_f32", "rstnet_rvq_encode_workspace", "rstnet_rvq_encode_f32",
@@ -109,10 +109,14 @@
     L.rstnet_tc_gemm_grid.argtypes = [vp, C.POINTER(i32), C.POINTER(i32), C.POINTER(i32)]
     L.rstnet_tc_gemm_create_ex.argtypes = [C.POINTER(TcGemmDesc), i32, C.POINTER(C.c_void_p)]
     L.rstnet_tc_gemm_kpair.argtypes = [vp, C.POINTER(i32)]
+    L.rstnet_tc_gemm_create_ex2.argtypes = [C.POINTER(TcGemmDesc), i32, i32, C.POINTER(C.c_void_p)]
+    L.rstnet_tc_gemm_occ2.argtypes = [vp, C.POINTER(i32)]
     L.rstnet_tc_resblock_create.argtypes = [C.POINTER(TcResblockDesc), C.POINTER(C.c_void_p)]
     L.rstnet_tc_resblock_run.argtypes = [vp, vp]
     L.rstnet_tc_resblock_destroy.argtypes = [vp]
     L.rstnet_tc_resblock_destroy.restype = None
+    L.rstnet_tc_resblock_create_ex.argtypes = [C.POINTER(TcResblockDesc), i32, C.POINTER(C.c_void_p)]
+    L.rstnet_tc_resblock_occ2.argtypes = [vp, C.POINTER(i32)]
     L.rstnet_tf32_split_f32.argtypes = [vp, vp, vp, i64, vp]
     L.rstnet_conv1d_cin1_f32.argtypes = [vp, i64, i64, vp, vp, vp, vp, i64, i64, i32, i32, i32, i32, i32, i32, vp]
     L.rstnet_conv1d_cout1_f32.argtypes = [vp, i64, i64, vp, vp, vp, i64, i32, i32, i32, i32, vp]
diff --git a/rstnet_b200/csrc/gemm_tc.cu b/rstnet_b200/csrc/gemm_tc.cu
--- a/rstnet_b200/csrc/gemm_tc.cu
+++ b/rstnet_b200/csrc/gemm_tc.cu
@@ -14,6 +14,8 @@
 constexpr int TC_CONSUMER_WARPS = 8;
 constexpr int TC_THREADS = 32 * TC_CONSUMER_WARPS + 32;
 constexpr int TC_CHUNK_STAGES = 4;
+constexpr int OCC2_MIN_K = 4, OCC2_MAX_K = 8;
+constexpr int RB_OCC2_MIN_ROUNDS = 2;
 
 struct TcParams {
   float* C;
@@ -30,17 +32,19 @@
   int pre_act, post_act, i_tiles;
   int m_tiles, n_tiles;
   int kpair;
+  int occ2;
 };
 
-template <int BN, int PREC>
+template <int BN, int PREC, bool OCC2 = false>
 struct TcCfg {
   static constexpr bool SPLIT = PREC == 0;
   static constexpr int B_BYTES = BN * 128;
   static constexpr int STAGE_BYTES = TC_A_BYTES + B_BYTES * (SPLIT ? 2 : 1);
-  static constexpr int STAGES = (200 * 1024 / STAGE_BYTES) > 8 ? 8 : (200 * 1024 / STAGE_BYTES);
+  static constexpr int STAGES = OCC2 ? 4 : (200 * 1024 / STAGE_BYTES) > 8 ? 8 : (200 * 1024 / STAGE_BYTES);
   static constexpr int SMEM_BYTES = STAGES * STAGE_BYTES + 1024  + 256 ;
   static constexpr int Q_PIECES = BN / 32;
   static_assert(STAGES % 2 == 0 && 2 * Q_PIECES <= STAGES, "K-pair rings and queue");
+  static_assert(!OCC2 || (BN == 32 && 2 * (SMEM_BYTES + 1024) <= 228 * 1024), "occupancy 2: BN = 32, two CTAs per SM");
 };
 
 __device__ __forceinline__ float tf32_rna(float x) {
@@ -98,11 +102,12 @@
   }
 }
 
-template <int BN, int PREC, bool PRE_ELU, bool KP>
-__global__ void __launch_bounds__(TC_THREADS, 1)
+template <int BN, int PREC, bool PRE_ELU, bool KP, bool OCC2>
+__global__ void __launch_bounds__(TC_THREADS, OCC2 ? 2 : 1)
 gemm_tc_kernel(const __grid_constant__ CUtensorMap tmA, const __grid_constant__ CUtensorMap tmW,
                const __grid_constant__ CUtensorMap tmWlo, const TcParams p) {
-  using Cfg = TcCfg<BN, PREC>;
+  static_assert(!(KP && OCC2), "K-pair and occupancy 2 exclude each other");
+  using Cfg = TcCfg<BN, PREC, OCC2>;
   constexpr int S = Cfg::STAGES;
   constexpr int CH = TC_CHUNK_STAGES;
   constexpr int NR = BN / 2;
@@ -183,8 +188,6 @@
   const int base = KP ? wg * R : 0;
   int pos = 0, ph = 0;
   for (int t = blockIdx.x; t < total_tiles; t += gridDim.x) {
-    const int nt = t % p.n_tiles, mt = t / p.n_tiles;
-    const int i0 = (mt % p.i_tiles) * bm, ot = mt / p.i_tiles, n0 = nt * BN;
 #pragma unroll
     for (int j = 0; j < NR; ++j) acc[j] = 0.f;
     for (int c = KP ? wg : 0; c < nch; c += KP ? 2 : 1) {
@@ -223,6 +226,8 @@
     }
     if (KP && !sender && nch % 2 == 0) take_queued();
     if (sender) continue;
+    const int nt = t % p.n_tiles, mt = t / p.n_tiles;
+    const int i0 = (mt % p.i_tiles) * bm, ot = mt / p.i_tiles, n0 = nt * BN;
 #pragma unroll
     for (int h = 0; h < 2; ++h) {
       const int i = i0 + r0 + 8 * h;
@@ -263,8 +268,6 @@
 }
 
 constexpr int RB_B_BYTES = 64 * 128;
-constexpr int RB_STAGE_BYTES = TC_A_BYTES + 2 * RB_B_BYTES;
-constexpr int RB_STAGES = 6;
 
 struct RbParams {
   float* out;
@@ -274,32 +277,39 @@
   int I_out, i_tiles, m_tiles;
 };
 
-template <int C>
+template <int C, bool OCC2 = false>
 struct RbCfg {
   static constexpr int N1 = C / 2;
   static constexpr int KCH = C / 32;
   static constexpr int P1 = 3 * KCH;
   static constexpr int NS = C / 64;
   static constexpr int K2 = N1 / 32;
+  static constexpr int PN = OCC2 ? 32 : 64;
+  static constexpr int STAGES = OCC2 ? 3 : 6;
+  static constexpr int B1_BYTES = OCC2 ? N1 * 128 : RB_B_BYTES;
+  static constexpr int STAGE_BYTES = TC_A_BYTES + 2 * B1_BYTES;
   static constexpr int H_BYTES = K2 * TC_A_BYTES;
-  static constexpr int SMEM_BYTES = RB_STAGES * RB_STAGE_BYTES + H_BYTES + 1024  + 256 ;
+  static constexpr int SMEM_BYTES = STAGES * STAGE_BYTES + H_BYTES + 1024  + 256 ;
   static constexpr bool ring_ok() {
     for (int j = 0; j < NS; ++j)
       for (int kc = 0; kc < KCH; ++kc)
-        if ((P1 + j) % RB_STAGES == (2 * KCH + kc) % RB_STAGES) return false;
-    return RB_STAGES >= KCH + NS;
+        if ((P1 + j) % STAGES == (2 * KCH + kc) % STAGES) return false;
+    return STAGES >= KCH + NS;
   }
   static_assert(ring_ok(), "ring too small for the held residual stages");
-  static_assert(K2 * 2 * RB_B_BYTES <= RB_STAGE_BYTES, "a phase-2 slice must fit one stage");
+  static_assert(K2 * 2 * RB_B_BYTES <= STAGE_BYTES, "a phase-2 slice must fit one stage");
+  static_assert(!OCC2 || (C == 64 && 2 * (SMEM_BYTES + 1024) <= 228 * 1024), "occupancy 2: C = 64, two CTAs per SM");
 };
 
-template <int C>
-__global__ void __launch_bounds__(TC_THREADS, 1)
+template <int C, bool OCC2>
+__global__ void __launch_bounds__(TC_THREADS, OCC2 ? 2 : 1)
 resblock_tc_kernel(const __grid_constant__ CUtensorMap tmY, const __grid_constant__ CUtensorMap tmW1,
                    const __grid_constant__ CUtensorMap tmW1lo, const __grid_constant__ CUtensorMap tmW2,
                    const __grid_constant__ CUtensorMap tmW2lo, const RbParams p) {
-  using Cfg = RbCfg<C>;
-  constexpr int S = RB_STAGES;
+  using Cfg = RbCfg<C, OCC2>;
+  constexpr int S = Cfg::STAGES;
+  constexpr int RB_STAGE_BYTES = Cfg::STAGE_BYTES;
+  constexpr int PN = Cfg::PN, NRP = PN / 2;
   constexpr int CH = TC_CHUNK_STAGES;
   constexpr int N1 = Cfg::N1, NR1 = N1 / 2, KCH = Cfg::KCH, P1 = Cfg::P1;
   extern __shared__ uint8_t smem_raw[];
@@ -336,7 +346,7 @@
           mbar_arrive_expect_tx(&full[s], TC_A_BYTES + 2 * N1 * 128);
           tma_load_3d(st, &tmY, &full[s], kc * TC_BKE, i0, ot + tap);
           tma_load_2d(st + TC_A_BYTES, &tmW1, &full[s], kit * TC_BKE, 0);
-          tma_load_2d(st + TC_A_BYTES + RB_B_BYTES, &tmW1lo, &full[s], kit * TC_BKE, 0);
+          tma_load_2d(st + TC_A_BYTES + Cfg::B1_BYTES, &tmW1lo, &full[s], kit * TC_BKE, 0);
         }
         for (int ns = 0; ns < Cfg::NS; ++ns, ++g) {
           const int s = g % S;
@@ -375,8 +385,8 @@
           uint32_t ah[4][4], al[4][4];
           tc_build_a<true, true>(st, a_row, a_sw, ah, al);
           wgmma_fence();
-          tc_mma_stage<N1, true>(d0, d1, ah, al, gmma_desc_sw128(st + TC_A_BYTES), gmma_desc_sw128(st + TC_A_BYTES + RB_B_BYTES),
-                                 u == 0);
+          tc_mma_stage<N1, true>(d0, d1, ah, al, gmma_desc_sw128(st + TC_A_BYTES),
+                                 gmma_desc_sw128(st + TC_A_BYTES + Cfg::B1_BYTES), u == 0);
           wgmma_commit();
           wgmma_wait<0>();
           __syncwarp();
@@ -410,46 +420,51 @@
       const int s = g % S;
       mbar_wait(&full[s], (g / S) & 1);
       const uint32_t st = smem0 + (uint32_t)(s * RB_STAGE_BYTES);
-      float acc[32], d0[32], d1[32];
-#pragma unroll
-      for (int j = 0; j < 32; ++j) d0[j] = d1[j] = 0.f;
-#pragma unroll
-      for (int kc = 0; kc < Cfg::K2; ++kc) {
-        uint32_t ah[4][4], al[4][4];
-        tc_build_a<true, false>(hs0 + (uint32_t)(kc * TC_A_BYTES), a_row, a_sw, ah, al);
-        const uint32_t wst = st + (uint32_t)(kc * 2 * RB_B_BYTES);
-        wgmma_fence();
-        tc_mma_stage<64, true>(d0, d1, ah, al, gmma_desc_sw128(wst), gmma_desc_sw128(wst + RB_B_BYTES), kc == 0);
-        wgmma_commit();
-        wgmma_wait<0>();
-      }
-      __syncwarp();
-      if (lane == 0) mbar_arrive(&empty[s]);
-      fence_acc(d0);
-      fence_acc(d1);
-#pragma unroll
-      for (int j = 0; j < 32; ++j) {
-        acc[j] = 0.f;
-        acc[j] += d0[j] + d1[j];
-      }
-#pragma unroll
-      for (int hh = 0; hh < 2; ++hh) {
-        const int r = r0 + 8 * hh;
-        const int i = i0 + r;
-        if (i >= p.I_out) continue;
-        float* orow = p.out + (long long)ot * p.o_o_stride + (long long)i * p.o_i_stride;
-#pragma unroll
-        for (int b = 0; b < 8; ++b) {
-          const int n = ns * 64 + 8 * b + 2 * tq;
-          const float2 bb = *reinterpret_cast<const float2*>(p.b2 + n);
-          float2 v = make_float2(acc[4 * b + 2 * hh], acc[4 * b + 2 * hh + 1]);
-          v.x += bb.x; v.y += bb.y;
-          const uint32_t cc = (uint32_t)(n % 32);
-          const int rs = (g_res + n / 32) % S;
-          const float2 rr = *reinterpret_cast<const float2*>(smem + rs * RB_STAGE_BYTES + r * 128 +
-                                                             (((cc >> 2) ^ (uint32_t)(r & 7)) << 4) + (cc & 3u) * 4u);
-          v.x += rr.x; v.y += rr.y;
-          *reinterpret_cast<float2*>(orow + n) = make_float2(act_tc(v.x, ACT_ELU), act_tc(v.y, ACT_ELU));
+#pragma unroll 1
+      for (int q = 0; q < 64 / PN; ++q) {
+        float acc[NRP], d0[NRP], d1[NRP];
+#pragma unroll
+        for (int j = 0; j < NRP; ++j) d0[j] = d1[j] = 0.f;
+#pragma unroll
+        for (int kc = 0; kc < Cfg::K2; ++kc) {
+          uint32_t ah[4][4], al[4][4];
+          tc_build_a<true, false>(hs0 + (uint32_t)(kc * TC_A_BYTES), a_row, a_sw, ah, al);
+          const uint32_t wst = st + (uint32_t)(kc * 2 * RB_B_BYTES + q * PN * 128);
+          wgmma_fence();
+          tc_mma_stage<PN, true>(d0, d1, ah, al, gmma_desc_sw128(wst), gmma_desc_sw128(wst + RB_B_BYTES), kc == 0);
+          wgmma_commit();
+          wgmma_wait<0>();
+        }
+        if (q == 64 / PN - 1) {
+          __syncwarp();
+          if (lane == 0) mbar_arrive(&empty[s]);
+        }
+        fence_acc(d0);
+        fence_acc(d1);
+#pragma unroll
+        for (int j = 0; j < NRP; ++j) {
+          acc[j] = 0.f;
+          acc[j] += d0[j] + d1[j];
+        }
+#pragma unroll(OCC2 ? 1 : 2)
+        for (int hh = 0; hh < 2; ++hh) {
+          const int r = r0 + 8 * hh;
+          const int i = i0 + r;
+          if (i >= p.I_out) continue;
+          float* orow = p.out + (long long)ot * p.o_o_stride + (long long)i * p.o_i_stride;
+#pragma unroll
+          for (int b = 0; b < PN / 8; ++b) {
+            const int n = ns * 64 + q * PN + 8 * b + 2 * tq;
+            const float2 bb = *reinterpret_cast<const float2*>(p.b2 + n);
+            float2 v = hh ? make_float2(acc[4 * b + 2], acc[4 * b + 3]) : make_float2(acc[4 * b], acc[4 * b + 1]);
+            v.x += bb.x; v.y += bb.y;
+            const uint32_t cc = (uint32_t)(n % 32);
+            const int rs = (g_res + n / 32) % S;
+            const float2 rr = *reinterpret_cast<const float2*>(smem + rs * RB_STAGE_BYTES + r * 128 +
+                                                               (((cc >> 2) ^ (uint32_t)(r & 7)) << 4) + (cc & 3u) * 4u);
+            v.x += rr.x; v.y += rr.y;
+            *reinterpret_cast<float2*>(orow + n) = make_float2(act_tc(v.x, ACT_ELU), act_tc(v.y, ACT_ELU));
+          }
         }
       }
       __syncwarp();
@@ -485,12 +500,12 @@
   int bn, prec;
 };
 
-template <int BN, int PREC, bool PRE_ELU, bool KP>
+template <int BN, int PREC, bool PRE_ELU, bool KP, bool OCC2 = false>
 static int tc_launch(const rstnet_tc_plan* pl, cudaStream_t st) {
-  using Cfg = TcCfg<BN, PREC>;
+  using Cfg = TcCfg<BN, PREC, OCC2>;
   static unsigned long long attr = 0;
-  smem_optin(gemm_tc_kernel<BN, PREC, PRE_ELU, KP>, Cfg::SMEM_BYTES, attr);
-  gemm_tc_kernel<BN, PREC, PRE_ELU, KP><<<pl->grid, TC_THREADS, Cfg::SMEM_BYTES, st>>>(pl->tmA, pl->tmW, pl->tmWlo, pl->p);
+  smem_optin(gemm_tc_kernel<BN, PREC, PRE_ELU, KP, OCC2>, Cfg::SMEM_BYTES, attr);
+  gemm_tc_kernel<BN, PREC, PRE_ELU, KP, OCC2><<<pl->grid, TC_THREADS, Cfg::SMEM_BYTES, st>>>(pl->tmA, pl->tmW, pl->tmWlo, pl->p);
   count_launch();
   return check_launch("gemm_tc");
 }
@@ -502,9 +517,38 @@
   return elu ? tc_launch<BN, PREC, true, false>(pl, st) : tc_launch<BN, PREC, false, false>(pl, st);
 }
 
+template <int PREC>
+static int tc_launch_occ2(const rstnet_tc_plan* pl, cudaStream_t st) {
+  return pl->p.pre_act == ACT_ELU ? tc_launch<32, PREC, true, false, true>(pl, st) : tc_launch<32, PREC, false, false, true>(pl, st);
+}
+
+template <typename Kernel>
+static int resident_ctas(Kernel* kernel, int smem) {
+  int n = 0;
+  if (cudaFuncSetAttribute(kernel, cudaFuncAttributeMaxDynamicSharedMemorySize, smem) != cudaSuccess ||
+      cudaOccupancyMaxActiveBlocksPerMultiprocessor(&n, kernel, TC_THREADS, smem) != cudaSuccess) {
+    cudaGetLastError();
+    return 0;
+  }
+  return n;
+}
+
+template <int PREC>
+static bool tc_occ2_fits(bool elu) {
+  constexpr int smem = TcCfg<32, PREC, true>::SMEM_BYTES;
+  return (elu ? resident_ctas(gemm_tc_kernel<32, PREC, true, false, true>, smem)
+              : resident_ctas(gemm_tc_kernel<32, PREC, false, false, true>, smem)) >= 2;
+}
+
 extern "C" int rstnet_tc_gemm_create_ex(const rstnet_tc_gemm_desc* d, int32_t kpair, rstnet_tc_plan** out) {
+  return rstnet_tc_gemm_create_ex2(d, kpair, -1, out);
+}
+
+extern "C" int rstnet_tc_gemm_create_ex2(const rstnet_tc_gemm_desc* d, int32_t kpair, int32_t occ2, rstnet_tc_plan** out) {
   RSTNET_REQUIRE(d && out, "tc_gemm_create: null argument");
   RSTNET_REQUIRE(kpair >= -1 && kpair <= 1, "tc_gemm_create: kpair must be -1 (auto), 0 or 1 (got %d)", kpair);
+  RSTNET_REQUIRE(occ2 >= -1 && occ2 <= 1, "tc_gemm_create: occ2 must be -1 (auto), 0 or 1 (got %d)", occ2);
+  RSTNET_REQUIRE(!(kpair == 1 && occ2 == 1), "tc_gemm_create: kpair and occ2 exclude each other");
   RSTNET_REQUIRE(d->A && d->W && d->C, "tc_gemm_create: null tensor pointer");
   RSTNET_REQUIRE(d->precision != 0 || d->W_lo, "tc_gemm_create: precision 0 (3xTF32) needs W_lo");
   RSTNET_REQUIRE(d->Kc > 0 && d->Kc % TC_BKE == 0, "tc_gemm_create: Kc (%d) must be a multiple of %d", d->Kc, TC_BKE);
@@ -529,12 +573,23 @@
     if (pl->bn == 64 && ((t32 + sms - 1) / sms) * 2 <= ((t64 + sms - 1) / sms) * 3) pl->bn = 32;
   }
   pl->prec = d->precision;
-  const int n_tiles = ceil_div(N, pl->bn);
+  int n_tiles = ceil_div(N, pl->bn);
   if (kpair < 0) {
     const long long total_k = (long long)d->taps * (d->Kc / TC_BKE);
     const long long t128 = (long long)i_tiles * d->O_out * n_tiles, t64 = (long long)ceil_div(d->I_out, TC_BM / 2) * d->O_out * n_tiles;
     const long long pair_k = (total_k + 2 * TC_CHUNK_STAGES - 1) / (2 * TC_CHUNK_STAGES) * TC_CHUNK_STAGES;
-    kpair = t128 <= sms && ((t64 + sms - 1) / sms) * pair_k < total_k;
+    kpair = occ2 != 1 && t128 <= sms && ((t64 + sms - 1) / sms) * pair_k < total_k;
+  }
+  if (kpair) occ2 = 0;
+  if (occ2 < 0) {
+    const long long total_k = (long long)d->taps * (d->Kc / TC_BKE);
+    const long long t32 = (long long)i_tiles * d->O_out * ceil_div(N, 32);
+    occ2 = t32 >= 2LL * sms && total_k >= OCC2_MIN_K && total_k <= OCC2_MAX_K;
+  }
+  if (occ2 && !(d->precision == 0 ? tc_occ2_fits<0>(d->pre_act == ACT_ELU) : tc_occ2_fits<1>(d->pre_act == ACT_ELU))) occ2 = 0;
+  if (occ2) {
+    pl->bn = 32;
+    n_tiles = ceil_div(N, 32);
   }
   const int bm = kpair ? TC_BM / 2 : TC_BM;
   {
@@ -577,11 +632,12 @@
   p.taps = d->taps; p.tap_di = d->tap_di; p.tap_do = d->tap_do; p.o_mul = d->o_mul; p.kchunks = d->Kc / TC_BKE;
   p.pre_act = d->pre_act; p.post_act = d->post_act;
   p.kpair = kpair;
+  p.occ2 = occ2;
   p.i_tiles = ceil_div(d->I_out, bm);
   p.m_tiles = p.i_tiles * d->O_out;
   p.n_tiles = n_tiles;
-  const long long tiles = (long long)p.m_tiles * p.n_tiles;
-  pl->grid = dim3((unsigned)(tiles < sms ? tiles : sms));
+  const long long tiles = (long long)p.m_tiles * p.n_tiles, ctas = (occ2 ? 2LL : 1LL) * sms;
+  pl->grid = dim3((unsigned)(tiles < ctas ? tiles : ctas));
   *out = pl;
   return 0;
 }
@@ -593,6 +649,7 @@
 extern "C" int rstnet_tc_gemm_run(const rstnet_tc_plan* pl, rstnet_stream_t stream) {
   RSTNET_REQUIRE(pl != nullptr, "tc_gemm_run: null plan");
   cudaStream_t st = (cudaStream_t)stream;
+  if (pl->p.occ2) return pl->prec == 0 ? tc_launch_occ2<0>(pl, st) : tc_launch_occ2<1>(pl, st);
   if (pl->prec == 0) return pl->bn == 64 ? tc_launch_mode<64, 0>(pl, st) : tc_launch_mode<32, 0>(pl, st);
   return pl->bn == 64 ? tc_launch_mode<64, 1>(pl, st) : tc_launch_mode<32, 1>(pl, st);
 }
@@ -604,6 +661,7 @@
   RbParams p;
   dim3 grid;
   int channels;
+  int occ2;
 };
 
 static int encode_2d(CUtensorMap* m, const float* base, int cols, int rows, int box_rows) {
@@ -616,7 +674,13 @@
 }
 
 extern "C" int rstnet_tc_resblock_create(const rstnet_tc_resblock_desc* d, rstnet_tc_resblock_plan** out) {
+  return rstnet_tc_resblock_create_ex(d, -1, out);
+}
+
+extern "C" int rstnet_tc_resblock_create_ex(const rstnet_tc_resblock_desc* d, int32_t occ2, rstnet_tc_resblock_plan** out) {
   RSTNET_REQUIRE(d && out, "tc_resblock_create: null argument");
+  RSTNET_REQUIRE(occ2 >= -1 && occ2 <= 1, "tc_resblock_create: occ2 must be -1 (auto), 0 or 1 (got %d)", occ2);
+  RSTNET_REQUIRE(occ2 != 1 || d->channels == 64, "tc_resblock_create: the occupancy-2 form is for 64 channels only");
   RSTNET_REQUIRE(d->Y && d->W1 && d->W1_lo && d->b1 && d->W2 && d->W2_lo && d->b2 && d->out, "tc_resblock_create: null pointer");
   const int Cc = d->channels;
   RSTNET_REQUIRE(Cc == 64 || Cc == 128, "tc_resblock_create: channels must be 64 or 128 (got %d)", Cc);
@@ -654,17 +718,21 @@
   p.i_tiles = ceil_div(d->I_out, TC_BM);
   p.m_tiles = p.i_tiles * d->O_out;
   const int sms = sm_count();
-  pl->grid = dim3((unsigned)(p.m_tiles < sms ? p.m_tiles : sms));
+  if (occ2 < 0) occ2 = Cc == 64 && p.m_tiles >= RB_OCC2_MIN_ROUNDS * sms;
+  if (occ2) occ2 = resident_ctas(resblock_tc_kernel<64, true>, RbCfg<64, true>::SMEM_BYTES) >= 2;
+  pl->occ2 = occ2;
+  const int ctas = (occ2 ? 2 : 1) * sms;
+  pl->grid = dim3((unsigned)(p.m_tiles < ctas ? p.m_tiles : ctas));
   *out = pl;
   return 0;
 }
 
-template <int Cc>
+template <int Cc, bool OCC2 = false>
 static int rb_launch(const rstnet_tc_resblock_plan* pl, cudaStream_t st) {
-  constexpr int smem = RbCfg<Cc>::SMEM_BYTES;
+  constexpr int smem = RbCfg<Cc, OCC2>::SMEM_BYTES;
   static unsigned long long attr = 0;
-  smem_optin(resblock_tc_kernel<Cc>, smem, attr);
-  resblock_tc_kernel<Cc><<<pl->grid, TC_THREADS, smem, st>>>(pl->tmY, pl->tmW1, pl->tmW1lo, pl->tmW2, pl->tmW2lo, pl->p);
+  smem_optin(resblock_tc_kernel<Cc, OCC2>, smem, attr);
+  resblock_tc_kernel<Cc, OCC2><<<pl->grid, TC_THREADS, smem, st>>>(pl->tmY, pl->tmW1, pl->tmW1lo, pl->tmW2, pl->tmW2lo, pl->p);
   count_launch();
   return check_launch("tc_resblock");
 }
@@ -672,6 +740,7 @@
 extern "C" int rstnet_tc_resblock_run(const rstnet_tc_resblock_plan* pl, rstnet_stream_t stream) {
   RSTNET_REQUIRE(pl != nullptr, "tc_resblock_run: null plan");
   cudaStream_t st = (cudaStream_t)stream;
+  if (pl->occ2) return rb_launch<64, true>(pl, st);
   return pl->channels == 64 ? rb_launch<64>(pl, st) : rb_launch<128>(pl, st);
 }
 
@@ -684,6 +753,16 @@
 extern "C" int rstnet_tc_gemm_kpair(const rstnet_tc_plan* pl, int32_t* on) {
   if (!pl) return 1;
   *on = pl->p.kpair;
+  return 0;
+}
+extern "C" int rstnet_tc_gemm_occ2(const rstnet_tc_plan* pl, int32_t* on) {
+  if (!pl) return 1;
+  *on = pl->p.occ2;
+  return 0;
+}
+extern "C" int rstnet_tc_resblock_occ2(const rstnet_tc_resblock_plan* pl, int32_t* on) {
+  if (!pl) return 1;
+  *on = pl->occ2;
   return 0;
 }
 
diff --git a/rstnet_b200/ops.py b/rstnet_b200/ops.py
--- a/rstnet_b200/ops.py
+++ b/rstnet_b200/ops.py
@@ -58,7 +58,7 @@
     def __init__(self, A, a_off, a_i_stride, a_o_stride, a_c_extent, a_i_extent, a_o_extent, W, Kc, C_, c_off, c_i_stride,
                  c_o_stride, I_out, O_out, *, taps=1, tap_di=0, tap_do=0, o_mul=1, bias=None, scale=None, R=None, r_off=0,
                  r_i_stride=0, r_o_stride=0, n_split=0, c_split_stride=0, r_split_stride=0, pre_act=ACT_NONE,
-                 post_act=ACT_NONE, precision=0, W_lo=None, C2=None, c2_off=0, act2=ACT_NONE):
+                 post_act=ACT_NONE, precision=0, W_lo=None, C2=None, c2_off=0, act2=ACT_NONE, kpair=-1, occ2=-1):
         _cuda(A, W, C_, bias, scale, R, W_lo)
         N, Ktot = W.shape
         if precision == 0 and W_lo is None:
@@ -85,7 +85,19 @@
         self.bytes = 4.0 * (a_c_extent * a_i_extent * in_rows + (2 if W_lo is not None else 1) * N * Ktot
                             + n_out * (2 if C2 is not None else 1) + (n_out if R is not None else 0))
         self._h = C.c_void_p()
-        _lib.check(_lib.lib().rstnet_tc_gemm_create(C.byref(d), C.byref(self._h)), "tc_gemm_create")
+        _lib.check(_lib.lib().rstnet_tc_gemm_create_ex2(C.byref(d), kpair, occ2, C.byref(self._h)), "tc_gemm_create")
+
+    @property
+    def kpair(self):
+        on = C.c_int32(0)
+        _lib.check(_lib.lib().rstnet_tc_gemm_kpair(self._h, C.byref(on)), "tc_gemm_kpair")
+        return on.value
+
+    @property
+    def occ2(self):
+        on = C.c_int32(0)
+        _lib.check(_lib.lib().rstnet_tc_gemm_occ2(self._h, C.byref(on)), "tc_gemm_occ2")
+        return on.value
 
     def run(self):
         _lib.check(_lib.lib().rstnet_tc_gemm_run(self._h, _stream()), "tc_gemm_run")
@@ -103,7 +115,7 @@
 class TcResblock:
 
     def __init__(self, Y, y_off, y_i_stride, y_o_stride, y_rows, I_out, O_out, W1, W1_lo, b1, W2, W2_lo, b2, out, out_off,
-                 out_i_stride, out_o_stride):
+                 out_i_stride, out_o_stride, *, occ2=-1):
         _cuda(Y, W1, W1_lo, b1, W2, W2_lo, b2, out)
         Cc = W2.shape[0]
         assert tuple(W1.shape) == (Cc // 2, 3 * Cc) and tuple(W2.shape) == (Cc, Cc // 2), (W1.shape, W2.shape)
@@ -121,7 +133,13 @@
         self.flops = 2.0 * n * (W1.numel() + W2.numel())
         self.bytes = 4.0 * (Cc * I_out * (O_out + 2) + 2 * (W1.numel() + W2.numel()) + b1.numel() + b2.numel() + n * Cc)
         self._h = C.c_void_p()
-        _lib.check(_lib.lib().rstnet_tc_resblock_create(C.byref(d), C.byref(self._h)), "tc_resblock_create")
+        _lib.check(_lib.lib().rstnet_tc_resblock_create_ex(C.byref(d), occ2, C.byref(self._h)), "tc_resblock_create")
+
+    @property
+    def occ2(self):
+        on = C.c_int32(0)
+        _lib.check(_lib.lib().rstnet_tc_resblock_occ2(self._h, C.byref(on)), "tc_resblock_occ2")
+        return on.value
 
     def run(self):
         _lib.check(_lib.lib().rstnet_tc_resblock_run(self._h, _stream()), "tc_resblock_run")
```

Measured after the change: 45540 (median of 6 runs). 1.02x the previous value.
